# istellartech/GELATO

Measured on AMD Instinct MI355X. Metric: residual+Jacobian evals/sec (and ms/eval), 6-phase x 64-node LGR mesh, higher is better.
Workload: dtype f64

## Files before the change

gelato_amd/csrc/gel_eval_kernel.h:

```cpp
#pragma once

namespace gel {

enum ParkSlot { PK_Q0 = 0, PK_Q1, PK_Q2, PK_Q3, PK_V0, PK_V1, PK_V2, PK_DJJ, PK_LV0, PK_LV1, PK_LV2,
                PK_FP0, PK_FP1, PK_FP2, PK_FP3, PK_FP4, PK_FP5, PK_FP6, PK_FP7, PK_COUNT };
constexpr int kStageLd = 17;
constexpr int kWaveLds = PK_COUNT * 64;
static_assert(kWaveLds >= 64 * kStageLd, "the MFMA staging tile must fit the wave's park region");
constexpr int kCoopStageOff = PK_LV0 * 64;
static_assert(kWaveLds - kCoopStageOff >= 64 * 11, "the cooperative hand-over area must fit behind the early park slots");
constexpr int kXldsPipeFrom = kLongPhaseFrom;
constexpr int kSlabRowsMax = 68, kPackRows = 36, kParkRes = (PK_LV2 + 1) * 64;
constexpr int kPipeSlabK = 8;
constexpr int wave_lds_doubles(bool jac, bool mfma, bool pack, bool split = false, bool longp = true) {
  return jac ? kWaveLds : (!mfma ? kParkRes : (split ? 64 * kStageLd  : (pack ? kParkRes + 4 * 64  : (longp ? 2 * 4 * kPipeSlabK * 11 + 64 * kPipeSlabK  : kSlabRowsMax * 11))));
}
static_assert(wave_lds_doubles(false, true, false, true) >= kParkRes, "residual-only split form: park over the result tile");
static_assert(wave_lds_doubles(false, true, true) >= 64 * 11 && wave_lds_doubles(false, true, false) >= 64 * 11 && wave_lds_doubles(false, true, false, false, false) >= 64 * 11, "hand-over area");
static_assert(wave_lds_doubles(false, true, true) >= kParkRes && wave_lds_doubles(false, true, false) >= kParkRes && wave_lds_doubles(false, true, false, false, false) >= kParkRes, "residual-only park");

constexpr int kSlotPT = 0, kSlotVM = 3, kSlotVP = 6;

#ifndef GEL_MIN_WAVES_PER_SIMD
#define GEL_MIN_WAVES_PER_SIMD 4
// ... 560 lines not shown
          __builtin_amdgcn_s_barrier();
        }
#undef GEL_PIPE_ROWS
#undef GEL_PIPE_A
#undef GEL_PIPE_WAIT
        lds_double* wg_lds = regions + kHO;
#pragma unroll
        for (int ct = 0; ct < 3; ct++) {
          const int c = 16 * ct + c16;
          const int vb = h7 ? c / 7 : c / 11, col = c - ncv * vb;
          if (c < ncols && (ct < 2 || !h7)) {
#pragma unroll
            for (int i = 0; i < 4; i++) wg_lds[vb * kWL + (16 * wv + kq + 4 * i) * 11 + col] = acc[ct][i];
          }
        }
        __syncthreads();
        if (ghost) return;
        lds_double* row = wave_lds + kHO + lane * 11;
        lm = row[0];
#pragma unroll
        for (int c = 0; c < 3; c++) { lr[c] = row[1 + c]; lv[c] = row[4 + c]; }
#pragma unroll
        for (int c = 0; c < 4; c++) lq[c] = row[7 + c];
      } else if (MFMA && csplit) {
        const int c16 = lane & 15, kq = lane >> 4;
        const double* bp = xm + ph.xa;
        int bs = 1;
        if (c16 >= 1 && c16 < 4) { bp = xr + 3 * ph.xa + (c16 - 1); bs = 3; }
        if (c16 >= 4 && c16 < 7) { bp = xv + 3 * ph.xa + (c16 - 4); bs = 3; }
        if (c16 >= 7) { bp = xq + 4 * ph.xa + ((c16 < 11) ? (c16 - 7) : 0); bs = 4; }
        gel_double4 acc1 = gel_double4{0.0, 0.0, 0.0, 0.0};
        const double* ap1 = P.Dst + (size_t)dsw * 4 + part * 64 + lane;
        const unsigned un = (unsigned)n, ubs = (unsigned)bs;
        if (tail1 && rb) {
          xl[0] = xm[ph.xa + n];
#pragma unroll
          for (int c = 0; c < 3; c++) { xl[1 + c] = xr[3 * (ph.xa + n) + c]; xl[4 + c] = xv[3 * (ph.xa + n) + c]; }
#pragma unroll
          for (int c = 0; c < 4; c++) xl[7 + c] = xq[4 * (ph.xa + n) + c];
        }
        constexpr int kSplitB = SPLITB, kSplitA = 4;
        if (n < kSlabRowsMax) {
          static_assert(!(SPLIT && MFMA && !JAC) || kSlabRowsMax * 11 <= kWL, "the state-row image must fit a wavefront's region");
          lds_double* img = wave_lds + (1 - part) * kWL;
          constexpr int kQRows = kSlabRowsMax / 4, kQ = kQRows * 11;
#pragma unroll
          for (int i = 0; i < (kQ + 63) / 64; i++) {
            const int e = lane + 64 * i;
            const int rl = (e * 373) >> 12, c = e - 11 * rl;
            const int r = kQRows * part + rl;
            if (e < kQ) {
              const int xr_ = ph.xa + min(r, n);
              const int off = (c == 0) ? xr_ : ((c < 4) ? M + 3 * xr_ + (c - 1) : ((c < 7) ? 4 * M + 3 * xr_ + (c - 4) : 7 * M + 4 * xr_ + (c - 7)));
              const double v = xb[off];
              img[r * 11 + c] = (r <= n) ? v : 0.0;
            }
          }
          double a1[kSplitA];
#pragma unroll
          for (int i = 0; i < kSplitA; i++) a1[i] = ap1[min(i, ksteps - 1) * 256];
          __syncthreads();
          const int bo = kq * 11 + ((c16 < 11) ? c16 : 0);
#pragma unroll
          for (int i = 0; i < kSlabRowsMax / 4; i++) {
            if (i < ksteps) {
              acc1 = __builtin_amdgcn_mfma_f64_16x16x4f64(a1[i % kSplitA], img[bo + 44 * i], acc1, 0, 0, 0);
              a1[i % kSplitA] = ap1[min(i + kSplitA, ksteps - 1) * 256];
            }
          }
        } else {
          for (int k0 = 0; k0 < ksteps; k0 += kSplitB) {
            double bl[kSplitB], a1[kSplitA];
#pragma unroll
            for (int i = 0; i < kSplitB; i++) bl[i] = bp[min(4u * (k0 + i) + kq, un) * ubs];
#pragma unroll
            for (int i = 0; i < kSplitA; i++) a1[i] = ap1[min(k0 + i, ksteps - 1) * 256];
#pragma unroll
            for (int i = 0; i < kSplitB; i++) {
              if (k0 + i < ksteps) {
                acc1 = __builtin_amdgcn_mfma_f64_16x16x4f64(a1[i % kSplitA], bl[i], acc1, 0, 0, 0);
                a1[i % kSplitA] = ap1[min(k0 + i + kSplitA, ksteps - 1) * 256];
              }
            }
          }
        }
        lds_double* lead_lds = wave_lds - part * kWL;
#pragma unroll
        for (int i = 0; i < 4; i++) lead_lds[(16 * part + kq + 4 * i) * kStageLd + c16] = acc1[i];
        __syncthreads();
        if (only_dx) return;
        if (rb) {
          lds_double* row = wave_lds + lane * kStageLd;
          lm = row[0];
#pragma unroll
          for (int c = 0; c < 3; c++) { lr[c] = row[1 + c]; lv[c] = row[4 + c]; }
#pragma unroll
          for (int c = 0; c < 4; c++) lq[c] = row[7 + c];
        }
      } else if (MFMA) {
        const int c16 = lane & 15, kq = lane >> 4;
        const double* bp = xm + ph.xa;
        int bs = 1;
        if (c16 >= 1 && c16 < 4) { bp = xr + 3 * ph.xa + (c16 - 1); bs = 3; }
        if (c16 >= 4 && c16 < 7) { bp = xv + 3 * ph.xa + (c16 - 4); bs = 3; }
        if (c16 >= 7) { bp = xq + 4 * ph.xa + ((c16 < 11) ? (c16 - 7) : 0); bs = 4; }
        gel_double4 acc[4];
#pragma unroll
        for (int t = 0; t < 4; t++) acc[t] = gel_double4{0.0, 0.0, 0.0, 0.0};
        const gel_double4* ap = reinterpret_cast<const gel_double4*>(P.Dsw) + (size_t)dsw * 1 + lane;
        const unsigned un = (unsigned)n, ubs = (unsigned)bs;
        if (tail1) {
          xl[0] = xm[ph.xa + n];
#pragma unroll
          for (int c = 0; c < 3; c++) { xl[1 + c] = xr[3 * (ph.xa + n) + c]; xl[4 + c] = xv[3 * (ph.xa + n) + c]; }
#pragma unroll
          for (int c = 0; c < 4; c++) xl[7 + c] = xq[4 * (ph.xa + n) + c];
        }
        constexpr int kSplitB = SPLITB, kSplitA = 2;
        for (int k0 = 0; k0 < ksteps; k0 += kSplitB) {
          double bl[kSplitB];
          gel_double4 a4[kSplitA];
#pragma unroll
          for (int i = 0; i < kSplitB; i++) bl[i] = bp[min(4u * (k0 + i) + kq, un) * ubs];
#pragma unroll
          for (int i = 0; i < kSplitA; i++) a4[i] = ap[min(k0 + i, ksteps - 1) * 64];
#pragma unroll
          for (int i = 0; i < kSplitB; i++) {
            if (k0 + i < ksteps) {
#pragma unroll
              for (int t = 0; t < 4; t++) acc[t] = __builtin_amdgcn_mfma_f64_16x16x4f64(a4[i % kSplitA][t], bl[i], acc[t], 0, 0, 0);
              a4[i % kSplitA] = ap[min(k0 + i + kSplitA, ksteps - 1) * 64];
            }
          }
        }
#pragma unroll
        for (int t = 0; t < 4; t++)
#pragma unroll
          for (int i = 0; i < 4; i++) wave_lds[(16 * t + kq + 4 * i) * kStageLd + c16] = acc[t][i];
        lds_double* row = wave_lds + lane * kStageLd;
        lm = row[0];
#pragma unroll
        for (int c = 0; c < 3; c++) { lr[c] = row[1 + c]; lv[c] = row[4 + c]; }
#pragma unroll
        for (int c = 0; c < 4; c++) lq[c] = row[7 + c];
      } else {
        const double* Dt = P.Dt + ph.doff + j;
        const double* pm = xm + ph.xa;
        const double* pr = xr + 3 * ph.xa;
        const double* pv = xv + 3 * ph.xa;
        const double* pq = xq + 4 * ph.xa;
        for (int i = 0; i <= n; i++) {
          const double d = Dt[(size_t)i * n];
          lm += d * pm[i];
#pragma unroll
          for (int c = 0; c < 3; c++) lr[c] += d * pr[3 * i + c];
#pragma unroll
          for (int c = 0; c < 3; c++) lv[c] += d * pv[3 * i + c];
#pragma unroll
          for (int c = 0; c < 4; c++) lq[c] += d * pq[4 * i + c];
        }
      }
    }
    GEL_TAKE_KNOT_TIMES();
#undef GEL_DX_TAIL_ACC
    if (SPLIT && tail1 && rb) {
      lm = __builtin_fma(dlast, xl[0], lm);
#pragma unroll
      for (int c = 0; c < 3; c++) { lr[c] = __builtin_fma(dlast, xl[1 + c], lr[c]); lv[c] = __builtin_fma(dlast, xl[4 + c], lv[c]); }
#pragma unroll
      for (int c = 0; c < 4; c++) lq[c] = __builtin_fma(dlast, xl[7 + c], lq[c]);
    }
    if (MFMA && !active) return;
    PARK_SET(PK_Q0, q[0]); PARK_SET(PK_Q1, q[1]); PARK_SET(PK_Q2, q[2]); PARK_SET(PK_Q3, q[3]);
    PARK_SET(PK_V0, ve[0]); PARK_SET(PK_V1, ve[1]); PARK_SET(PK_V2, ve[2]);
    if (JAC) PARK_SET(PK_DJJ, djj);
    if (rb) { PARK_SET(PK_LV0, lv[0]); PARK_SET(PK_LV1, lv[1]); PARK_SET(PK_LV2, lv[2]); }
    if (!ref0_done) {
      if (rb && !ph.engine_on) m0 = xm[ph.xa];
      if (rb && ph.hold) {
#pragma unroll
        for (int c = 0; c < 4; c++) q0[c] = xq[4 * ph.xa + c];
      }
    }

    if (JAC && lead) {
      if (coo) {
        const double sc = -(P.kpt * (tf - to));
        double* d_ = P.coo_full + GEL_COO_BASE(CG_PV) + (size_t)3 * j0;
#pragma unroll
        for (int i = 0; i < 3; i++) d_[(cw8 == 512) ? 64 * i + lane : 3 * lane + i] = sc;
      } else if (j == 0) EMIT_AT(packed ? (ph.K - sub_hi) * cw8 : ph.K * n * 8, -(P.kpt * (tf - to)));
      {
        const double pt[3] = {ve[0] * P.kpt, ve[1] * P.kpt, ve[2] * P.kpt};
        EMIT_GROUP(3, kSlotPT, pt, CG_PT, 0, true, true);
      }
    }
    if (!ph.hold && lead) {
      double fq[4];
      quat_rate(q, u0, u1, P.uu, fq);
      if (rb) {
        double cq[4];
#pragma unroll
        for (int c = 0; c < 4; c++) cq[c] = lq[c] - fq[c] * (tf - to) * hT;
        RSTORE_ROWS(wave_lds + kTileOff, 4, rs_q, cq);
      }
      if (JAC && ph.q_fd) {
        double f[4];
#pragma unroll
        for (int k = 0; k < 4; k++) {
          double qp[4];
#pragma unroll
          for (int c = 0; c < 4; c++) qp[c] = (k == c) ? (q[c] + dx) : q[c];
          quat_rate(qp, u0, u1, P.uu, f);
          const int c0 = (k < 2) ? 2 : 0;
          EMIT(ph.s_qq + 2 * k, FDQ(f[c0], fq[c0]));
          EMIT(ph.s_qq + 2 * k + 1, FDQ(f[c0 + 1], fq[c0 + 1]));
        }
#pragma unroll 1
        for (int k = 0; k < 2; k++) {
          quat_rate(q, (k == 0) ? u0 + dx : u0, (k == 1) ? u1 + dx : u1, P.uu, f);
#pragma unroll
          for (int c = 0; c < 4; c++) EMIT(ph.s_qq + 8 + 4 * k + c, FDQ(f[c], fq[c]));
        }
#pragma unroll
        for (int c = 0; c < 4; c++) EMIT(ph.s_qq + 16 + c, fq[c] * hT);
      } else if (JAC) {
        const double hS = (tf - to) * ut / 2.0;
        const double d2r = 0.017453292519943295769;
        EMIT(ph.s_qq + 0, 0.5 * ((u0 * P.uu) * d2r) * hS);
        EMIT(ph.s_qq + 1, 0.5 * ((u1 * P.uu) * d2r) * hS);
        const double kq = 0.5 * (P.uu * d2r) * hS;
        if (coo) {
          const double C0 = kq * q[0], C1 = kq * q[1], C2 = kq * q[2], C3 = kq * q[3];
          const double u0v[4] = {C2, C3, -C0, -C1}, u1v[4] = {C3, -C2, C1, -C0};
          EMIT_GROUP(4, 0, u0v, CG_QU, 0, false, true);
          EMIT_GROUP(4, 0, u1v, CG_QU, 1, false, true);
        } else {
          EMIT(ph.s_qq + 2, -(kq * q[0]));
          EMIT(ph.s_qq + 3, kq * q[1]);
          EMIT(ph.s_qq + 4, kq * q[2]);
          EMIT(ph.s_qq + 5, kq * q[3]);
        }
        {
          const double qt[4] = {fq[0] * hT, fq[1] * hT, fq[2] * hT, fq[3] * hT};
          EMIT_GROUP(4, ph.s_qq + 6, qt, CG_QT, 0, true, true);
        }
      }
    }
    if (rb) {
      double cm;
      if (ph.engine_on) {
        const double rh = ph.mf_um * (tf - to) * ut / 2.0;
        cm = lm - rh;
      } else {
        cm = me - m0;
      }
      RSTORE(rs_m + gn, cm);
      GEL_CHK(cm);
      {
        double cp[3];
        const double kpos = P.kpt * (tf - to);
#pragma unroll
        for (int c = 0; c < 3; c++) cp[c] = lr[c] - ve[c] * kpos;
        RSTORE_ROWS(wave_lds + kTileOff, 3, rs_p, cp);
      }
      if (ph.hold) {
        double cq[4];
#pragma unroll
        for (int c = 0; c < 4; c++) cq[c] = q[c] - q0[c];
        RSTORE_ROWS(wave_lds + kTileOff, 4, rs_q, cq);
      }
    }
  }
  asm volatile("" ::: "memory");

  double fc[3];
  {
    const double tn = tau * (tf - to) / 2 + (tf + to) / 2;
    const double inv_m = frcp(me * P.um);

#define GEL_QUAT_CLOSED(Tval)                                                                                          \
  do {                                                                                                                 \
    const double kq_ = ((Tval) * inv_m) * (inv_uv * fds);                                                              \
    const double q_[4] = {PARK_GET(PK_Q0), PARK_GET(PK_Q1), PARK_GET(PK_Q2), PARK_GET(PK_Q3)};                         \
    _Pragma("unroll") for (int k = 0; k < 4; k++) {                                                                    \
      const double dl_ = (q_[k] + dx) - q_[k];                                                                         \
      const double a_ = (k < 2) ? -(dl_ * kq_) : dl_ * kq_;    \
      const double b_ = -2.0 * (dl_ * kq_);                                                                            \
      const double vq_[3] = {(2.0 * q_[k] + dl_) * a_,                                                                 \
                             q_[3 - k] * b_,                                    \
                             ((k & 1) ? q_[k ^ 2] : -q_[k ^ 2]) * b_};        \
      EMIT_GROUP(3, ph.s_vq + 3 * k, vq_, CG_VQ, k, false, true);                                                      \
    }                                                                                                                  \
  } while (0)
#define GEL_MASS_CLOSED(tm_)                                                                                           \
  do {                                                                                                                 \
          \
    const double e_ = (fresh_product(me + dx, P.um) - fresh_product(me, P.um)) * inv_m;                                \
    const double k_ = (e_ * (1.0 - e_ * (1.0 - e_))) * (inv_uv * fds);                                                 \
    const double vm_[3] = {(tm_)[0] * k_, (tm_)[1] * k_, (tm_)[2] * k_};                                               \
    EMIT_GROUP(3, kSlotVM, vm_, CG_VM, 0, false, true);                                                                \
  } while (0)
    if (ph.air) {
      EarthHalf eh{1.0, 0.0};
      bool have_eh = false;
#define GEL_NEED_EARTH_ANGLE(wn_, we_)                                                                                 \
  do {                                                                                                                 \
    if (!have_eh && __builtin_amdgcn_ballot_w64(!((wn_) == 0.0 && (we_) == 0.0)) != 0) {                                \
      int jl_ = jc;                                                                                                    \
      if (AERO) asm volatile("" : "+v"(jl_));    \
      const double tau_ = P.tau[ph.toff + jl_];                                                                        \
      const EarthAngle e_ = earth_angle(tau_ * (tf - to) / 2 + (tf + to) / 2);                                         \
      eh.ch = e_.ch; eh.sh = e_.sh; have_eh = true;                                                                    \
    }                                                                                                                  \
  } while (0)
      PosCentreTail pt;
      double cen_rho = 0.0, cen_P = 0.0, cen_inv_a = 0.0;
      double dir2 = 0.0;
      EarthHalf aeh{1.0, 0.0};
      bool have_aeh = false;
#ifndef GEL_AEH
#define GEL_AEH aeh
#endif
#ifndef GEL_X_NOPOS
#define GEL_X_NOPOS 0
#endif
#ifndef GEL_X_NOQUAT
#define GEL_X_NOQUAT 0
#endif
#ifndef GEL_X_NOVEL
#define GEL_X_NOVEL 0
#endif
      const bool aero_on = AERO && akinds != 0;
      const bool a_need_alpha = AERO && (akinds & 5) != 0;
#define GEL_AERO_NEED_EA(wn_, we_)                                                                                     \
  do {                                                                                                                 \
    if (!have_aeh && __builtin_amdgcn_ballot_w64(!((wn_) == 0.0 && (we_) == 0.0)) != 0) {                               \
      int jl_ = jc;                                                                                                    \
      asm volatile("" : "+v"(jl_));    \
      const double tau_ = P.tau[ph.toff + jl_];                                                                        \
      const EarthAngle e_ = earth_angle((tau_ * (tf - to) / 2 + (tf + to) / 2) * P.ut);                                \
      aeh.ch = e_.ch; aeh.sh = e_.sh; have_aeh = true;                                                                 \
    }                                                                                                                  \
  } while (0)
#define GEL_AERO_FETCH()                                                                                               \
  const int ab_[3] = {load_const(&aph->base[0]), load_const(&aph->base[1]), load_const(&aph->base[2])};                \
  const double ax_[3] = {load_const(&aph->ilx[0]), load_const(&aph->ilx[1]), load_const(&aph->ilx[2])};                \
  const int n8_ = 8 * n, j08_ = 8 * j0
#define GEL_AERO_ENTRY(blk, col, a_, nv2_, d_, ind_, rho_, okl_, a_cc, a_ac, a_qc, a_isc, a_ok)                         \
  do {                                                                                                                 \
    double t_ = 0.0, dq_ = 0.0, qp_ = 0.0;                                                                             \
    const double ac_ = a_ac;                                                                                           \
    {                                                                                                                  \
      const double qc_ = a_qc;                                                                                         \
      qp_ = 0.5 * (rho_) * (nv2_);                                                                                     \
      dq_ = qp_ - qc_;                                                                                                 \
      if (a_need_alpha) {                                                                                              \
        const double cp_ = aero_cos(a_, nv2_, d_, ind_);                                                               \
        const bool okd_ = aero_dalpha(cp_, nv2_, a_cc, a_isc, a_ok, t_);                                               \
        if (__builtin_amdgcn_ballot_w64(!okd_) != 0) {                                                                 \
          const double t2_ = aero_acos(cp_, nv2_) - ac_;                                                               \
          t_ = okd_ ? t_ : t2_;                                                                                        \
        }                                                                                                              \
      }                                                                                                                \
    }                                                                                                                  \
    _Pragma("unroll") for (int kind = 0; kind < 3; kind++) {                                                           \
      if ((blk) == 2 && kind == 1) continue;                             \
      const double df_ = (kind == 0) ? t_ : ((kind == 1) ? dq_ : qp_ * t_ + dq_ * ac_);                                \
      const double gv = -(df_ * ax_[kind]);                                                                            \
      if (okl_) AEMIT(ab_[kind] + (((blk) == 0 ? 1 : ((blk) == 1 ? 4 : 7)) + (col)) * n8_ + j08_, gv);                 \
    }                                                                                                                  \
  } while (0)
#if GEL_CA_CACHE
      Bracket ca_br = no_bracket();
#define GEL_CA_BRACKET (JAC ? &ca_br : (Bracket*)nullptr)
#else
#define GEL_CA_BRACKET nullptr
#endif
      struct ParkSink { lds_double* park; GEL_DEV void put(int i, double v) const { if (!(AERO && (i == PCS_P || i == PCS_IH))) park[(PK_FP0 + i) * 64] = v; } };
      constexpr int PK_ACC = PK_FP0 + PCS_P, PK_AAC = PK_FP0 + PCS_IH, PK_AQC = PK_LV2;
      static_assert(PCS_COUNT == 8 && PK_FP7 == PK_FP0 + 7, "PosCentre's early members fill FP0-7");
      {
        PosPart pp;
        double v[3], w[3], F[3], dir[3];
        const double r[3] = {fresh_product(re[0], P.up), fresh_product(re[1], P.up), fresh_product(re[2], P.up)};
        if (JAC) pp = pos_part<true, ParkSink>(r, tb, P.barC20, nullptr, ParkSink{park}, &pt);
        else pp = pos_part(r, tb, P.barC20);
        if (__builtin_amdgcn_ballot_w64(!(pp.wn == 0.0 && pp.we == 0.0)) != 0) {
          const EarthAngle e0 = earth_angle(tn);
          eh.ch = e0.ch; eh.sh = e0.sh; have_eh = true;
          if (aero_on) PARK_SET(PK_ACC, tn);
        }
        const EarthAngle ea = full_angle(eh);
        wind_eci_or_calm(r, ea, pp.shp, pp.chp, pp.inv_p, pp.wn, pp.we, w);
#pragma unroll
        for (int c = 0; c < 3; c++) v[c] = PARK_GET(PK_V0 + c) * P.uv;
        aero_force(r, v, pp.rho, pp.inv_a, ea, w, ph.area, tb, F, GEL_CA_BRACKET);
#define GEL_T (ph.thrust - ph.nozzle * pp.P)
#define GEL_TDC(name) const double name[3] = {GEL_T * dir[0], GEL_T * dir[1], GEL_T * dir[2]}
        {
          const double q[4] = {PARK_GET(PK_Q0), PARK_GET(PK_Q1), PARK_GET(PK_Q2), PARK_GET(PK_Q3)};
          thrust_dir(q, dir);
        }
        double tm[3];
        {
          GEL_TDC(Tdc);
          accel_parts(Tdc, F, inv_m, pp.g, inv_uv, tm, fc);
        }
        if (rb) {
#ifndef GEL_RES_XPOSE_VEL_AIR
#define GEL_RES_XPOSE_VEL_AIR 1
#endif
          if (!JAC || GEL_RES_XPOSE_VEL_AIR) {
            double cv[3];
#pragma unroll
            for (int c = 0; c < 3; c++) cv[c] = PARK_GET(PK_LV0 + c) - fc[c] * (tf - to) * hT;
            RSTORE_ROWS(wave_lds + PK_LV0 * 64, 3, rs_v, cv);
          } else {
#pragma unroll
            for (int c = 0; c < 3; c++) {
              const double cv = PARK_GET(PK_LV0 + c) - fc[c] * (tf - to) * hT;
              RSTORE(rs_v + 3 * gn + c, cv);
              GEL_CHK(cv);
            }
          }
        }
        if (JAC) {
          asm volatile("" ::: "memory");
          PARK_SET(PK_LV0, pp.shp); PARK_SET(PK_LV1, pp.chp);
          if (!AERO) PARK_SET(PK_LV2, pp.inv_p);
        }
        if (JAC && lead && !P.fd_recompute) GEL_MASS_CLOSED(tm);
        if (JAC && ph.air_fd && (SPLIT && P.split_vel ? !lead : lead)) {
          double f[3];
          {
            const double djj = PARK_GET(PK_DJJ);
#pragma unroll
            for (int k = 0; k < 3; k++) {
              if (SPLIT && P.split_vel && k != part - 1) continue;
              double vp[3], Fp[3];
#pragma unroll
              for (int c = 0; c < 3; c++) vp[c] = ((k == c) ? (PARK_GET(PK_V0 + c) + dx) : PARK_GET(PK_V0 + c)) * P.uv;
              const double r[3] = {fresh_product(re[0], P.up), fresh_product(re[1], P.up), fresh_product(re[2], P.up)};
              aero_force(r, vp, pp.rho, pp.inv_a, ea, w, ph.area, tb, Fp, GEL_CA_BRACKET);
              GEL_TDC(Tdc);
              accel(Tdc, Fp, inv_m, pp.g, inv_uv, f);
#pragma unroll
              for (int c = 0; c < 3; c++) EMIT(ph.s_vv + 3 * k + c, ((c == k) ? djj : 0.0) + FDQ(f[c], fc[c]));
            }
          }
        }
        if (JAC && lead) {
          double f[3];
          if (!P.fd_recompute) {
            GEL_QUAT_CLOSED(GEL_T);
          } else if (P.fd_recompute) {
            const double q[4] = {PARK_GET(PK_Q0), PARK_GET(PK_Q1), PARK_GET(PK_Q2), PARK_GET(PK_Q3)};
#pragma unroll 1
            for (int k = 0; k < 4; k++) {
              double qp[4];
#pragma unroll
              for (int c = 0; c < 4; c++) qp[c] = (k == c) ? (q[c] + dx) : q[c];
              double dp[3];
              thrust_dir(qp, dp);
              const double Td[3] = {GEL_T * dp[0], GEL_T * dp[1], GEL_T * dp[2]};
              accel(Td, F, inv_m, pp.g, inv_uv, f);
#pragma unroll
              for (int c = 0; c < 3; c++) EMIT(ph.s_vq + 3 * k + c, FDQ(f[c], fc[c]));
            }
            GEL_TDC(Tdc);
            accel(Tdc, F, frcp((me + dx) * P.um), pp.g, inv_uv, f);
#pragma unroll
            for (int c = 0; c < 3; c++) EMIT(kSlotVM + c, FDQ(f[c], fc[c]));
          }
          if (!ph.t_fd) {
            const double vt[3] = {fc[0] * hT, fc[1] * hT, fc[2] * hT};
            EMIT_GROUP(3, ph.s_vt, vt, CG_VT, 0, true, true);
          }
        }
        if (aero_on) {
          asm volatile("" ::: "memory");
          const double ra[3] = {fresh_product(re[0], P.up), fresh_product(re[1], P.up), fresh_product(re[2], P.up)};
          double va[3], wa[3], a0[3];
#pragma unroll
          for (int c = 0; c < 3; c++) va[c] = PARK_GET(PK_V0 + c) * P.uv;
          if (have_eh) {
            const EarthAngle e1 = earth_angle(PARK_GET(PK_ACC) * P.ut);
            aeh.ch = e1.ch; aeh.sh = e1.sh; have_aeh = true;
          }
          if (have_aeh) {
            PosCentre pcx;
            double wn_, we_, p_, ip_, ih_;
            pos_centre_tail(pt, pp.rho, pp.P, tb, pcx, wn_, we_);
            geodetic_p_ih(ra[0], ra[1], ra[2], p_, ip_, ih_);
            wind_eci(ra, full_angle(GEL_AEH), PARK_GET(PK_LV0), PARK_GET(PK_LV1), ip_, wn_, we_, wa);
          } else {
            wa[0] = 0.0; wa[1] = 0.0; wa[2] = 0.0;
          }
          const double nv2 = aero_vair2(ra, va, wa, a0);
          const double ind = frsqrt(fmax(dir[0] * dir[0] + dir[1] * dir[1] + dir[2] * dir[2], 1.0e-300));
          const double cc = a_need_alpha ? aero_cos(a0, nv2, dir, ind) : 0.0;
          const double alpha_c = a_need_alpha ? aero_acos(cc, nv2) : 0.0;
          const double qdyn_c = 0.5 * pp.rho * nv2;
          double sc, isc;
          fsqrt_rsqrt(fmax((1.0 - cc) * (1.0 + cc), 1.0e-300), sc, isc);
          const bool centre_ok = (cc <= 1.0) && (nv2 >= 1.0e-12) && (sc > 1.0e-6);
          GEL_AERO_FETCH();
          const double ail_[3] = {load_const(&aph->il[0]), load_const(&aph->il[1]), load_const(&aph->il[2])};
#pragma unroll
          for (int kind = 0; kind < 3; kind++) {
            const double il = ail_[kind];
            const double cv = 1.0 - ((kind == 0) ? alpha_c : (kind == 1) ? qdyn_c : qdyn_c * alpha_c) * il;
            AEMIT(ab_[kind] + j08_, cv);
            GEL_CHK(cv);
          }
          if (a_need_alpha && !GEL_X_NOQUAT) {
            const double q[4] = {PARK_GET(PK_Q0), PARK_GET(PK_Q1), PARK_GET(PK_Q2), PARK_GET(PK_Q3)};
#pragma unroll
            for (int c = 0; c < 4; c++) {
              double qp[4], dp[3];
#pragma unroll
              for (int d = 0; d < 4; d++) qp[d] = (d == c) ? q[d] + dx : q[d];
              thrust_dir(qp, dp);
              const double indp = frsqrt(fmax(dp[0] * dp[0] + dp[1] * dp[1] + dp[2] * dp[2], 1.0e-300));
              GEL_AERO_ENTRY(2, c, a0, nv2, dp, indp, pp.rho, true, cc, alpha_c, qdyn_c, isc, centre_ok);
              __builtin_amdgcn_sched_barrier(0);
            }
          }
#pragma unroll
          for (int c = 0; c < (GEL_X_NOVEL ? 0 : 3); c++) {
            double vp[3], a[3];
#pragma unroll
            for (int d = 0; d < 3; d++) vp[d] = ((d == c) ? PARK_GET(PK_V0 + d) + dx : PARK_GET(PK_V0 + d)) * P.uv;
            const double nv2p = aero_vair2(ra, vp, wa, a);
            GEL_AERO_ENTRY(1, c, a, nv2p, dir, ind, pp.rho, true, cc, alpha_c, qdyn_c, isc, centre_ok);
            __builtin_amdgcn_sched_barrier(0);
          }
          PARK_SET(PK_ACC, cc); PARK_SET(PK_AAC, centre_ok ? alpha_c : -alpha_c); PARK_SET(PK_AQC, qdyn_c);
        }
        if (JAC) {
          asm volatile("" ::: "memory");
          PARK_SET(PK_Q0, fc[0]); PARK_SET(PK_Q1, fc[1]); PARK_SET(PK_Q2, fc[2]); PARK_SET(PK_Q3, dir[0]); PARK_SET(PK_DJJ, dir[1]);
          dir2 = dir[2];
          cen_rho = pp.rho; cen_P = pp.P; cen_inv_a = pp.inv_a;
        }
#undef GEL_TDC
#undef GEL_T
      }
      if (JAC && (!SPLIT || part)) {
        const int k0 = SPLIT ? part - 1 : 0, k1 = SPLIT ? part : 3;
#define GEL_POS_SWEEP_F(rp, pq, f_)                                                                           \
  do {                                                                                                        \
    double wq_[3], Fp_[3];                                                                                    \
    GEL_NEED_EARTH_ANGLE((pq).wn, (pq).we);                                                                   \
    const EarthAngle ea = full_angle(eh);                                                                     \
    wind_eci_or_calm(rp, ea, (pq).shp, (pq).chp, (pq).inv_p, (pq).wn, (pq).we, wq_);                          \
    const double vq_[3] = {PARK_GET(PK_V0) * P.uv, PARK_GET(PK_V1) * P.uv, PARK_GET(PK_V2) * P.uv};           \
    aero_force(rp, vq_, (pq).rho, (pq).inv_a, ea, wq_, ph.area, tb, Fp_, GEL_CA_BRACKET);                     \
    const double Tp_ = ph.thrust - ph.nozzle * (pq).P;                                                        \
    const double Td_[3] = {Tp_ * PARK_GET(PK_Q3), Tp_ * PARK_GET(PK_DJJ), Tp_ * dir2};                        \
    accel(Td_, Fp_, inv_m, (pq).g, inv_uv, f_);                                                               \
  } while (0)
#define GEL_POS_SWEEP_EMIT(kk, f_, okl_)                                                                      \
  do {                                                                                                        \
    const double vp_[3] = {FDQ((f_)[0], PARK_GET(PK_Q0)), FDQ((f_)[1], PARK_GET(PK_Q1)), FDQ((f_)[2], PARK_GET(PK_Q2))}; \
    EMIT_GROUP(3, kSlotVP + 3 * (kk), vp_, CG_VP, kk, false, okl_);                                           \
  } while (0)
#define GEL_AERO_POS(kk, rp, pq, okl_)                                                                        \
  do {                                                                                                        \
    double wq_[3], a_[3];                                                                                     \
    GEL_AERO_NEED_EA((pq).wn, (pq).we);                                                                       \
    wind_eci_or_calm(rp, full_angle(GEL_AEH), (pq).shp, (pq).chp, (pq).inv_p, (pq).wn, (pq).we, wq_);             \
    const double vq_[3] = {PARK_GET(PK_V0) * P.uv, PARK_GET(PK_V1) * P.uv, PARK_GET(PK_V2) * P.uv};           \
    const double nv2_ = aero_vair2(rp, vq_, wq_, a_);                                                         \
    const double dd_[3] = {PARK_GET(PK_Q3), PARK_GET(PK_DJJ), dir2};                                          \
    const double ind_ = frsqrt(fmax(dd_[0] * dd_[0] + dd_[1] * dd_[1] + dd_[2] * dd_[2], 1.0e-300));          \
    const double cc_ = PARK_GET(PK_ACC);                                                                      \
    double sc_, isc_;                                                                                         \
    fsqrt_rsqrt(fmax((1.0 - cc_) * (1.0 + cc_), 1.0e-300), sc_, isc_);                                        \
    const double acs_ = PARK_GET(PK_AAC);    \
    GEL_AERO_FETCH();                                                                                         \
    GEL_AERO_ENTRY(0, kk, a_, nv2_, dd_, ind_, (pq).rho, okl_, cc_, fabs(acs_), PARK_GET(PK_AQC), isc_, !__builtin_signbit(acs_)); \
  } while (0)
#define GEL_LOAD_POS_CENTRE(pc, pcv)                                                                                   \
  PosCentre pc;                                                                                                        \
  pc.ihy = PARK_GET(PK_FP0 + PCS_IHY);                                                                                 \
  pc.sl = PARK_GET(PK_FP0 + PCS_SL); pc.cl = PARK_GET(PK_FP0 + PCS_CL); pc.icl = PARK_GET(PK_FP0 + PCS_ICL);           \
  pc.N = PARK_GET(PK_FP0 + PCS_N); pc.G = PARK_GET(PK_FP0 + PCS_G);                                                    \
  PosPart pcv;                                                                                                         \
  pcv.rho = cen_rho; pcv.P = cen_P; pcv.inv_a = cen_inv_a;                                                             \
  pcv.shp = PARK_GET(PK_LV0); pcv.chp = PARK_GET(PK_LV1);                                                              \
  if (AERO) {                                                                                                          \
    geodetic_p_ih(fresh_product(re[0], P.up), fresh_product(re[1], P.up), fresh_product(re[2], P.up), pc.p, pcv.inv_p, pc.ih); \
  } else {                                                                                                             \
    pc.p = PARK_GET(PK_FP0 + PCS_P); pc.ih = PARK_GET(PK_FP0 + PCS_IH); pcv.inv_p = PARK_GET(PK_LV2);                  \
  }                                                                                                                    \
  pos_centre_tail(pt, cen_rho, cen_P, tb, pc, pcv.wn, pcv.we)
        unsigned todo = 0;
        unsigned long long coo_okm = 0;
        if (P.fd_recompute) {
          todo = ((1u << k1) - 1u) & ~((1u << k0) - 1u);
        } else {
#pragma unroll
          for (int k = k0; k < k1; k++) {
            asm volatile("" ::: "memory");
            GEL_LOAD_POS_CENTRE(pc, pcv);
            const double r[3] = {fresh_product(re[0], P.up), fresh_product(re[1], P.up), fresh_product(re[2], P.up)};
            double rp[3];
#pragma unroll
            for (int c = 0; c < 3; c++) rp[c] = (k == c) ? (re[c] + dx) * P.up : r[c];
            const double dlt = (k == 0) ? rp[0] - r[0] : ((k == 1) ? rp[1] - r[1] : rp[2] - r[2]);
            PosPart pq;
            const bool ok = pos_delta(r, k, dlt, pcv, pc, tb, pq);
            if (coo) coo_okm = __builtin_amdgcn_ballot_w64(ok);
            if (__builtin_amdgcn_ballot_w64(!ok) != 0) {
              todo |= 1u << k;
              if (__builtin_amdgcn_ballot_w64(ok) == 0) continue;
            }
            gravity_eci(rp, P.barC20, pq.g);
            double f[3];
            GEL_POS_SWEEP_F(rp, pq, f);
            GEL_POS_SWEEP_EMIT(k, f, ok);
            if (aero_on && !GEL_X_NOPOS) GEL_AERO_POS(k, rp, pq, ok);
          }
        }
        if (todo) {
#pragma unroll 1
          for (int k = k0; k < k1; k++) {
            if (!((todo >> k) & 1u)) continue;
            asm volatile("" ::: "memory");
            double rp[3];
#pragma unroll
            for (int c = 0; c < 3; c++) rp[c] = fresh_product((k == c) ? re[c] + dx : re[c], P.up);
            bool ok = false;
            if (!P.fd_recompute && coo) {
              ok = ((coo_okm >> lane) & 1ull) != 0;
            } else if (!P.fd_recompute) {
              GEL_LOAD_POS_CENTRE(pc, pcv);
              const double r[3] = {fresh_product(re[0], P.up), fresh_product(re[1], P.up), fresh_product(re[2], P.up)};
              const double dlt = (k == 0) ? rp[0] - r[0] : ((k == 1) ? rp[1] - r[1] : rp[2] - r[2]);
              PosPart pd;
              ok = pos_delta(r, k, dlt, pcv, pc, tb, pd);
            }
            asm volatile("" ::: "memory");
            PosPart pq = pos_part(rp, tb, P.barC20);
            double f[3];
            GEL_POS_SWEEP_F(rp, pq, f);
            GEL_POS_SWEEP_EMIT(k, f, !ok);
            if (aero_on && !GEL_X_NOPOS) GEL_AERO_POS(k, rp, pq, !ok);
          }
        }
#undef GEL_AERO_POS
#undef GEL_LOAD_POS_CENTRE
#undef GEL_NEED_EARTH_ANGLE
#undef GEL_AERO_NEED_EA
#undef GEL_AERO_ENTRY
#undef GEL_AERO_FETCH
#undef GEL_POS_SWEEP_F
#undef GEL_POS_SWEEP_EMIT
      }
      if (JAC && lead && ph.t_fd) {
        asm volatile("" ::: "memory");
        const double fcc[3] = {PARK_GET(PK_Q0), PARK_GET(PK_Q1), PARK_GET(PK_Q2)};
        int jl2 = jc;
        if (AERO) asm volatile("" : "+v"(jl2));
        const double tau2 = P.tau[ph.toff + jl2];
        {
          const double r[3] = {fresh_product(re[0], P.up), fresh_product(re[1], P.up), fresh_product(re[2], P.up)};
          const PosPart p2 = pos_part(r, tb, P.barC20);
          const double T2 = ph.thrust - ph.nozzle * p2.P;
          PARK_SET(PK_FP0, p2.shp); PARK_SET(PK_FP1, p2.chp); PARK_SET(PK_FP2, p2.inv_p); PARK_SET(PK_FP3, p2.wn); PARK_SET(PK_FP4, p2.we);
          PARK_SET(PK_FP5, p2.rho); PARK_SET(PK_FP6, p2.inv_a);
          PARK_SET(PK_LV0, p2.g[0]); PARK_SET(PK_LV1, p2.g[1]); PARK_SET(PK_LV2, p2.g[2]);
          PARK_SET(PK_Q0, T2 * PARK_GET(PK_Q3)); PARK_SET(PK_Q1, T2 * PARK_GET(PK_DJJ)); PARK_SET(PK_Q2, T2 * dir2);
        }
#pragma unroll 1
        for (int k = 0; k < 2; k++) {
          asm volatile("" ::: "memory");
          const double to_p = (k == 0) ? to + dx : to;
          const double tf_p = (k == 1) ? tf + dx : tf;
          const double tnp = tau2 * (tf_p - to_p) / 2 + (tf_p + to_p) / 2;
          const EarthAngle eq = earth_angle(tnp);
          double wq[3], Fp[3], f[3];
          const double rq[3] = {re[0] * P.up, re[1] * P.up, re[2] * P.up};
          wind_eci_or_calm(rq, eq, PARK_GET(PK_FP0), PARK_GET(PK_FP1), PARK_GET(PK_FP2), PARK_GET(PK_FP3), PARK_GET(PK_FP4), wq);
          const double vq[3] = {PARK_GET(PK_V0) * P.uv, PARK_GET(PK_V1) * P.uv, PARK_GET(PK_V2) * P.uv};
          aero_force(rq, vq, PARK_GET(PK_FP5), PARK_GET(PK_FP6), eq, wq, ph.area, tb, Fp, GEL_CA_BRACKET);
          const double Tq[3] = {PARK_GET(PK_Q0), PARK_GET(PK_Q1), PARK_GET(PK_Q2)};
          const double gq[3] = {PARK_GET(PK_LV0), PARK_GET(PK_LV1), PARK_GET(PK_LV2)};
          accel(Tq, Fp, inv_m, gq, inv_uv, f);
#pragma unroll
          for (int c = 0; c < 3; c++)
            EMIT(ph.s_vt + 3 * k + c, (fcc[c] * (tf - to) - f[c] * (tf_p - to_p)) * fdt);
        }
      }
    } else {
      const double T = ph.thrust;
      double dir[3];
      {
        const double q[4] = {PARK_GET(PK_Q0), PARK_GET(PK_Q1), PARK_GET(PK_Q2), PARK_GET(PK_Q3)};
        thrust_dir(q, dir);
      }
      const double Td[3] = {T * dir[0], T * dir[1], T * dir[2]};
      double gc[3];
      {
        const double r[3] = {re[0] * P.up, re[1] * P.up, re[2] * P.up};
        gravity_eci(r, P.barC20, gc);
      }
      double tm[3];
#pragma unroll
      for (int c = 0; c < 3; c++) { tm[c] = Td[c] * inv_m; fc[c] = (tm[c] + gc[c]) * inv_uv; }
      if (rb) {
        double cv[3];
#pragma unroll
        for (int c = 0; c < 3; c++) cv[c] = PARK_GET(PK_LV0 + c) - fc[c] * (tf - to) * hT;
        RSTORE_ROWS(wave_lds + PK_LV0 * 64, 3, rs_v, cv);
      }
      if (JAC) {
        double f[3];
        if (!P.fd_recompute) {
          GEL_MASS_CLOSED(tm);
        } else {
          accel_noair(Td, frcp((me + dx) * P.um), gc, inv_uv, f);
#pragma unroll
          for (int c = 0; c < 3; c++) EMIT(kSlotVM + c, FDQ(f[c], fc[c]));
        }
#pragma unroll
        for (int k = 0; k < 3; k++) {
          double r[3], gp[3];
#pragma unroll
          for (int c = 0; c < 3; c++) r[c] = ((k == c) ? (re[c] + dx) : re[c]) * P.up;
          gravity_eci(r, P.barC20, gp);
          accel_noair(Td, inv_m, gp, inv_uv, f);
          const double vp[3] = {FDQ(f[0], fc[0]), FDQ(f[1], fc[1]), FDQ(f[2], fc[2])};
          EMIT_GROUP(3, kSlotVP + 3 * k, vp, CG_VP, k, false, true);
        }
        if (!P.fd_recompute) {
          GEL_QUAT_CLOSED(T);
        } else {
          const double q[4] = {PARK_GET(PK_Q0), PARK_GET(PK_Q1), PARK_GET(PK_Q2), PARK_GET(PK_Q3)};
#pragma unroll 1
          for (int k = 0; k < 4; k++) {
            double qp[4];
#pragma unroll
            for (int c = 0; c < 4; c++) qp[c] = (k == c) ? (q[c] + dx) : q[c];
            double dp[3];
            thrust_dir(qp, dp);
            const double Tp[3] = {T * dp[0], T * dp[1], T * dp[2]};
            accel_noair(Tp, inv_m, gc, inv_uv, f);
#pragma unroll
            for (int c = 0; c < 3; c++) EMIT(ph.s_vq + 3 * k + c, FDQ(f[c], fc[c]));
          }
        }
        {
          const double vt[3] = {fc[0] * hT, fc[1] * hT, fc[2] * hT};
          EMIT_GROUP(3, ph.s_vt, vt, CG_VT, 0, true, true);
        }
      }
    }
  }
#undef EMIT_GROUP
#undef GEL_COO_EMIT
#undef GEL_COO_BASE
#undef EMIT
#undef GEL_CA_BRACKET
#undef GEL_QUAT_CLOSED
#undef GEL_MASS_CLOSED
#undef AEMIT
#undef EMIT_AT
#undef RSTORE
#undef RSTORE_ROWS
#undef RSTORE_LINE
#undef xpose
#undef FDQ
#undef GEL_CHK
#undef GEL_UNI
#undef GEL_TAKE_KNOT_TIMES
#undef PARK_GET
#undef PARK_SET
  if (bad) *(volatile int32_t*)P.flag = 1;
}

__device__ __forceinline__ void signal_done(const ProblemDev& P) {
  if (!P.done_flag) return;
  __threadfence_system();
  __syncthreads();
  if (threadIdx.x == 0) {
    const int old = __hip_atomic_fetch_add(P.done_ctr, 1, __ATOMIC_ACQ_REL, __HIP_MEMORY_SCOPE_AGENT);
    if (old == P.done_total - 1) {
      __hip_atomic_store(P.done_ctr, 0, __ATOMIC_RELAXED, __HIP_MEMORY_SCOPE_AGENT);
      __hip_atomic_store(P.done_flag, P.done_seq, __ATOMIC_RELEASE, __HIP_MEMORY_SCOPE_SYSTEM);
    }
  }
}

template <bool JAC, bool MFMA, bool SPLIT = false, bool PACK = false, bool LONGP = true, bool NTS = true, bool AERO = false>
__global__ __launch_bounds__(kBlock, (!JAC && PACK) ? GEL_MIN_WAVES_PER_SIMD_RES : ((JAC && PACK) ? GEL_MIN_WAVES_PER_SIMD_PACKJAC : GEL_MIN_WAVES_PER_SIMD)) void eval_kernel(ProblemDev P, int B, const double* __restrict__ x,
                                                      double* __restrict__ res, double* __restrict__ jvar) {
  eval_body<JAC, MFMA, SPLIT, PACK, 9, LONGP, NTS, AERO>(P, B, x, res, jvar, blockIdx.x);
  if constexpr (SPLIT) signal_done(P);
}

}
```

gelato_amd/csrc/gel_kernels.hip:

```cpp
#include <hip/hip_runtime.h>

#include "gel_tables.h"

#include "gel_eval_kernel.h"
namespace gel {

constexpr int kExpandGroup = 8;
__global__ __launch_bounds__(kBlock) void expand_kernel(long long nnz, long long V, int B, const double* __restrict__ cval,
                                                        const int32_t* __restrict__ src,
                                                        const double* __restrict__ jvar, double* __restrict__ full) {
  const int b0 = blockIdx.y * kExpandGroup;
  const int nb = min(kExpandGroup, B - b0);
  const bool even = (nnz & 1) == 0;
  for (long long i = 2 * ((long long)blockIdx.x * kBlock + threadIdx.x); i < nnz; i += 2LL * gridDim.x * kBlock) {
    const bool two = i + 1 < nnz;
    const int s0 = src[i], s1 = two ? src[i + 1] : -1;
    const double c0 = (s0 == -1) ? cval[i] : 0.0, c1 = (two && s1 == -1) ? cval[i + 1] : 0.0;
    const int g0 = (s0 >= 0) ? s0 : -2 - s0, g1 = (s1 >= 0) ? s1 : -2 - s1;
    for (int g = 0; g < nb; g++) {
      const double* jv = jvar + (size_t)(b0 + g) * V;
      double* out = full + (size_t)(b0 + g) * nnz + i;
      const double v0 = (s0 == -1) ? c0 : ((s0 >= 0) ? jv[g0] : -jv[g0]);
      const double v1 = (s1 == -1) ? c1 : ((s1 >= 0) ? jv[g1] : -jv[g1]);
      if (two && (even || ((b0 + g) & 1) == 0)) {
        typedef double gel_d2 __attribute__((ext_vector_type(2)));
        __builtin_nontemporal_store(gel_d2{v0, v1}, reinterpret_cast<gel_d2*>(out));
      } else {
        __builtin_nontemporal_store(v0, out);
        if (two) __builtin_nontemporal_store(v1, out + 1);
      }
    }
  }
}

__global__ __launch_bounds__(kBlock) void update_full_kernel(long long nnz, long long V, int nvar, int B, const int32_t* __restrict__ vdst,
                                                             const int32_t* __restrict__ vsrc, const double* __restrict__ jvar,
                                                             double* __restrict__ full) {
  const int i = blockIdx.x * kBlock + threadIdx.x;
  if (i >= nvar) return;
  const int d = vdst[i], s = vsrc[i];
  const int g = (s >= 0) ? s : -2 - s;
  for (int b = blockIdx.y; b < B; b += gridDim.y) {
    const double v = jvar[(size_t)b * V + g];
    full[(size_t)b * nnz + d] = (s >= 0) ? v : -v;
  }
}
__global__ __launch_bounds__(kBlock) void update_lines_kernel(long long nnz, long long V, int nlines, int B, const int32_t* __restrict__ vline,
                                                              const int32_t* __restrict__ src, const double* __restrict__ cval,
                                                              const double* __restrict__ jvar, double* __restrict__ full) {
  const int t = blockIdx.x * kBlock + threadIdx.x;
  if (t >= 8 * nlines) return;
  const long long i = 8LL * vline[t >> 3] + (t & 7);
  const int s = src[i];
  const double c = (s == -1) ? cval[i] : 0.0;
  const int g = (s >= 0) ? s : -2 - s;
  for (int b = blockIdx.y; b < B; b += gridDim.y) {
    double v = c;
    if (s != -1) { const double w = jvar[(size_t)b * V + g]; v = (s >= 0) ? w : -w; }
    __builtin_nontemporal_store(v, full + (size_t)b * nnz + i);
  }
}
__global__ __launch_bounds__(kBlock) void fill_full_kernel(long long nnz, int B, const double* __restrict__ cval, double* __restrict__ full) {
  for (long long i = (long long)blockIdx.x * kBlock + threadIdx.x; i < nnz; i += (long long)gridDim.x * kBlock) {
    const double c = cval[i];
    for (int b = blockIdx.y; b < B; b += gridDim.y) __builtin_nontemporal_store(c, full + (size_t)b * nnz + i);
  }
}

__global__ void perturb_local_kernel(int nloc, double dx, const double* __restrict__ x, const int32_t* __restrict__ colmap,
                                     double* __restrict__ Xp) {
  const long long t = (long long)blockIdx.x * blockDim.x + threadIdx.x;
  if (t >= (long long)(nloc + 1) * nloc) return;
  const int row = (int)(t / nloc), col = (int)(t - (long long)row * nloc);
  double v = x[colmap[col]];
  if (row == col + 1) v += dx;
  Xp[t] = v;
}

__global__ void quotient_local_kernel(int nloc, int nres, int roff, int nrows, double dx, const double* __restrict__ res,
                                      double* __restrict__ J, long long ldJ, int row0, const int32_t* __restrict__ colmap) {
  __shared__ double tile[32][33];
  const int c0 = blockIdx.x * 32, r0 = blockIdx.y * 32;
  for (int k = threadIdx.y; k < 32; k += blockDim.y) {
    const int c = c0 + k, r = r0 + threadIdx.x;
    if (c < nloc && r < nrows) tile[k][threadIdx.x] = res[(size_t)(c + 1) * nres + roff + r];
  }
  __syncthreads();
  for (int k = threadIdx.y; k < 32; k += blockDim.y) {
    const int r = r0 + k, c = c0 + threadIdx.x;
    if (c < nloc && r < nrows) J[(size_t)(row0 + r) * ldJ + (colmap ? colmap[c] : c)] = (tile[threadIdx.x][k] - res[roff + r]) / dx;
  }
}

struct RhsArgs {
  int n, Kw, Kc;
  const double *mass_e, *pos_e, *vel_e, *quat, *t, *tables;
  double thrust, area, nozzle, um, up, uv, barC20;
  double* out;
};

__global__ void rhs_vel_air_kernel(RhsArgs A) {
  extern __shared__ double lds[];
  ProblemDev P{};
  P.Kw = A.Kw; P.Kc = A.Kc; P.tables = A.tables;
  const Tables tb = stage_tables(P, lds);
  const int i = blockIdx.x * blockDim.x + threadIdx.x;
  if (i >= A.n) return;
  const double m = A.mass_e[i] * A.um;
  const double r[3] = {A.pos_e[3 * i] * A.up, A.pos_e[3 * i + 1] * A.up, A.pos_e[3 * i + 2] * A.up};
  const double v[3] = {A.vel_e[3 * i] * A.uv, A.vel_e[3 * i + 1] * A.uv, A.vel_e[3 * i + 2] * A.uv};
  const double q[4] = {A.quat[4 * i], A.quat[4 * i + 1], A.quat[4 * i + 2], A.quat[4 * i + 3]};
  const PosPart pp = pos_part(r, tb, A.barC20);
  const EarthAngle ea = earth_angle(A.t[i]);
  double w[3], F[3], dir[3], f[3];
  wind_eci(r, ea, pp.shp, pp.chp, pp.inv_p, pp.wn, pp.we, w);
  aero_force(r, v, pp.rho, pp.inv_a, ea, w, A.area, tb, F);
  thrust_dir(q, dir);
  const double T = A.thrust - A.nozzle * pp.P;
  const double Td[3] = {T * dir[0], T * dir[1], T * dir[2]};
  accel(Td, F, 1.0 / m, pp.g, 1.0 / A.uv, f);
  for (int c = 0; c < 3; c++) A.out[3 * i + c] = f[c];
}

__global__ void rhs_vel_noair_kernel(RhsArgs A) {
  const int i = blockIdx.x * blockDim.x + threadIdx.x;
  if (i >= A.n) return;
  const double m = A.mass_e[i] * A.um;
  const double r[3] = {A.pos_e[3 * i] * A.up, A.pos_e[3 * i + 1] * A.up, A.pos_e[3 * i + 2] * A.up};
  const double q[4] = {A.quat[4 * i], A.quat[4 * i + 1], A.quat[4 * i + 2], A.quat[4 * i + 3]};
  double dir[3], g[3], f[3];
  thrust_dir(q, dir);
  gravity_eci(r, A.barC20, g);
  const double Td[3] = {A.thrust * dir[0], A.thrust * dir[1], A.thrust * dir[2]};
  accel_noair(Td, 1.0 / m, g, 1.0 / A.uv, f);
  for (int c = 0; c < 3; c++) A.out[3 * i + c] = f[c];
}

__global__ void rhs_quat_kernel(int n, const double* quat, const double* u_e, double unit_u, double* out) {
  const int i = blockIdx.x * blockDim.x + threadIdx.x;
  if (i >= n) return;
  const double q[4] = {quat[4 * i], quat[4 * i + 1], quat[4 * i + 2], quat[4 * i + 3]};
  double dq[4];
  quat_rate(q, u_e[2 * i], u_e[2 * i + 1], unit_u, dq);
  for (int c = 0; c < 4; c++) out[4 * i + c] = dq[c];
}

__global__ void point_kernel(int kind, int n, const double* in, const double* aux, int aux_rows, double* out) {
  extern __shared__ double lds[];
  const int naux = (kind == 5 || kind == 10) ? 3 * aux_rows + 2 * (aux_rows - 1)
                   : (kind == 6 || kind == 9) ? 2 * aux_rows + (aux_rows - 1) : (kind == 0 ? kAtmDoubles : 0);
  for (int i = threadIdx.x; i < naux; i += blockDim.x) lds[i] = aux[i];
  __syncthreads();
  const int i = blockIdx.x * blockDim.x + threadIdx.x;
  if (i >= n) return;
  switch (kind) {
    case 0: {
      const double h = geopotential_altitude(in[i]);
      const Air a = atmosphere(h, lds);
      out[5 * i] = h; out[5 * i + 1] = a.T; out[5 * i + 2] = a.P; out[5 * i + 3] = a.rho; out[5 * i + 4] = a.a;
    } break;
    case 1: {
      double lat, sl, cl, p, ip;
      geodetic_lat_p(in[3 * i], in[3 * i + 1], in[3 * i + 2], lat, p, ip);
      geodetic_sincos_p(in[3 * i], in[3 * i + 1], in[3 * i + 2], sl, cl, p, ip);
      const double lon = atan2(in[3 * i + 1], in[3 * i]);
      out[3 * i] = lat * 180.0 / kPi; out[3 * i + 1] = lon * 180.0 / kPi;
      out[3 * i + 2] = geodetic_alt_from(p, sl, cl);
    } break;
    case 2: {
      const double r[3] = {in[3 * i], in[3 * i + 1], in[3 * i + 2]};
      double g[3];
      gravity_eci(r, aux[0], g);
      out[3 * i] = g[0]; out[3 * i + 1] = g[1]; out[3 * i + 2] = g[2];
    } break;
    case 3: {
      const double* a = in + 6 * i;
      const double r[3] = {a[0], a[1], a[2]};
      double sl, cl, p, ip, w[3];
      geodetic_sincos_p(r[0], r[1], r[2], sl, cl, p, ip);
      const EarthAngle ea = earth_angle(a[3]);
      double chp, irt;
      fsqrt_rsqrt(0.5 * (1.0 + cl), chp, irt);
      wind_eci(r, ea, (0.5 * sl) * irt, chp, ip, a[4], a[5], w);
      out[3 * i] = w[0]; out[3 * i + 1] = w[1]; out[3 * i + 2] = w[2];
    } break;
    case 4: {
      const double* a = in + 7 * i;
      double s, c;
      sincos(kOmega * a[6], &s, &c);
      const double d0 = a[0] - (0.0 * a[5] - kOmega * a[4]);
      const double d1 = a[1] - (kOmega * a[3] - 0.0 * a[5]);
      const double d2 = a[2] - (0.0 * a[4] - 0.0 * a[3]);
      out[3 * i] = d0 * c + d1 * s; out[3 * i + 1] = -d0 * s + d1 * c; out[3 * i + 2] = d2;
    } break;
    case 5: {
      double wn, we;
      wind_ned2(in[i], lds, lds + 3 * aux_rows, aux_rows, wn, we);
      out[3 * i] = wn; out[3 * i + 1] = we; out[3 * i + 2] = 0.0;
    } break;
    case 6: out[i] = interp_tab(in[i], lds, lds + 2 * aux_rows, aux_rows, 2, 1); break;
    case 7: {
      const double a = in[2 * i], b = in[2 * i + 1];
      out[4 * i] = fsqrt(a); out[4 * i + 1] = sqrt(a); out[4 * i + 2] = fdiv(a, b); out[4 * i + 3] = a / b;
    } break;
    case 8: {
      double s1, c1, s2, c2;
      fsincos(in[2 * i], &s1, &c1);
      sincos(in[2 * i], &s2, &c2);
      out[6 * i] = s1; out[6 * i + 1] = c1; out[6 * i + 2] = s2; out[6 * i + 3] = c2;
      out[6 * i + 4] = flog_ratio(in[2 * i + 1]); out[6 * i + 5] = log(in[2 * i + 1]);
    } break;
    case 9: {
      Bracket br = no_bracket();
      for (int k = 0; k < 8; k++) out[8 * i + k] = interp_tab_cached(in[8 * i + k], lds, lds + 2 * aux_rows, aux_rows, 2, 1, br);
    } break;
    case 10: {
      Bracket2 br = no_bracket2();
      for (int k = 0; k < 8; k++) {
        double wn, we;
        wind_ned2_cached(in[8 * i + k], lds, lds + 3 * aux_rows, aux_rows, wn, we, br);
        out[16 * i + 2 * k] = wn; out[16 * i + 2 * k + 1] = we;
      }
    } break;
    case 11: {
      double o[4];
      quatmult(in + 8 * i, in + 8 * i + 4, o);
      for (int c = 0; c < 4; c++) out[4 * i + c] = o[c];
    } break;
    case 12: {
      double o[3];
      quatrot(in + 7 * i, in + 7 * i + 4, o);
      for (int c = 0; c < 3; c++) out[3 * i + c] = o[c];
    } break;
    case 13: {
      const double* q = in + 4 * i;
      out[7 * i] = q[0]; out[7 * i + 1] = -q[1]; out[7 * i + 2] = -q[2]; out[7 * i + 3] = -q[3];
      double d[3];
      thrust_dir(q, d);
      for (int c = 0; c < 3; c++) out[7 * i + 4 + c] = d[c];
    } break;
    case 14: out[2 * i] = fexp(in[i]); out[2 * i + 1] = exp(in[i]); break;
    default: break;
  }
}

struct AeroPos {
  double rho;
  double wn, we;
  double shp, chp, inv_p;
};

GEL_DEV AeroPos aero_pos_part(const double r[3], const Tables& tb) {
  AeroPos o;
  double lat, p, sl, cl;
  geodetic_lat_p(r[0], r[1], r[2], lat, p, o.inv_p);
  fsincos(lat, &sl, &cl);
  const double h = geopotential_altitude(geodetic_alt_from(p, sl, cl));
  wind_ned2(h, tb.wind, tb.winds, tb.Kw, o.wn, o.we);
  double irt;
  fsqrt_rsqrt(0.5 * (1.0 + cl), o.chp, irt);
  o.shp = (0.5 * sl) * irt;
  o.rho = atmosphere(h, tb.atm).rho;
  return o;
}

GEL_DEV double aero_vair(const double r[3], const double v[3], const EarthAngle& ea, const double w[3], double a[3]) {
  const double d0 = v[0] + kOmega * r[1], d1 = v[1] - kOmega * r[0];
  const double e0 = d0 * ea.c + d1 * ea.s, e1 = -d0 * ea.s + d1 * ea.c;
  a[0] = (e0 * ea.c - e1 * ea.s) - w[0]; a[1] = (e0 * ea.s + e1 * ea.c) - w[1]; a[2] = v[2] - w[2];
  return sqrt(a[0] * a[0] + a[1] * a[1] + a[2] * a[2]);
}

GEL_DEV double aero_alpha(const double a[3], double nv, const double q[4]) {
  double dir[3];
  thrust_dir(q, dir);
  const double nd = sqrt(dir[0] * dir[0] + dir[1] * dir[1] + dir[2] * dir[2]);
  const double c_alpha = (a[0] / nv) * (dir[0] / nd) + (a[1] / nv) * (dir[1] / nd) + (a[2] / nv) * (dir[2] / nd);
  return (c_alpha > 1.0) ? 0.0 : ((nv < 1e-6) ? 0.0 : acos(c_alpha));
}

struct AeroOut {
  double* con[3];
  double* jac[3];
  int32_t nrows[3];
  int64_t ld;
  int32_t sm;
};

#ifndef GEL_AERO_UNROLL
#define GEL_AERO_UNROLL 1
#endif
constexpr int kAeroWaves = 4;
enum { AP_ILIM = 0, AP_AC = 3, AP_QC, AP_CC, AP_IS, AP_IND, AP_W = 8, AP_A0 = 11, AP_DIR = 14, AP_RHO = 17, AP_NV2 = 18, AP_INTS = 19,
       kAeroParkSlots = 25 };
typedef __attribute__((address_space(3))) int lds_int;
typedef __attribute__((address_space(3))) double lds_f64;
template <bool ROLES, bool WIDE = false, bool SM = false>
__device__ __forceinline__ void aero_body(const ProblemDev P, int nnodes, const AeroNodeDev* __restrict__ nodes, int tiles, int B,
                                          const double* __restrict__ x, const AeroOut O, const unsigned vblk) {
  extern __shared__ double lds[];
  const Tables tb = stage_tables(P, lds);
  const int lane = (int)(threadIdx.x & 63);
  const int sw = ROLES ? (int)(threadIdx.x >> 6) : -1;
  const long long wid = ROLES ? (long long)vblk : (long long)vblk * kAeroWaves + __builtin_amdgcn_readfirstlane((int)(threadIdx.x >> 6));
  const bool flat = !ROLES && !WIDE && tiles == 0;
  int b, ni_raw;
  bool live;
  if (WIDE) {
    const long long total = (long long)B * nnodes, f = wid * 64 + lane;
    if (wid * 64 >= total) return;
    live = f < total;
    const long long fc = live ? f : total - 1;
    b = (int)(fc / nnodes);
    ni_raw = live ? (int)(fc - (long long)b * nnodes) : nnodes;
  } else if (flat) {
    const long long total = (long long)B * nnodes, f0 = wid * 64;
    if (f0 >= total) return;
    const int b0 = (int)(f0 / nnodes), r0 = (int)(f0 - (long long)b0 * nnodes);
    const bool wrap = r0 + lane >= nnodes;
    live = f0 + lane < total;
    b = live ? (wrap ? b0 + 1 : b0) : b0;
    ni_raw = live ? (wrap ? r0 + lane - nnodes : r0 + lane) : nnodes;
  } else {
    if (wid >= (long long)B * tiles) return;
    b = (int)(wid / tiles);
    ni_raw = (int)(wid - (long long)b * tiles) * 64 + lane;
    live = ni_raw < nnodes;
  }
  const int ni = live ? ni_raw : nnodes - 1;
  const AeroNodeDev Nd = nodes[ni];
  const PhaseDev& ph = P.phases[Nd.phase];
  const double* xb = x + (size_t)b * P.nvars;
  const int M = P.M, N = P.N, xi = ph.xa + Nd.k;
  const double dx = P.dx;
  double re[3];
#pragma unroll
  for (int c = 0; c < 3; c++) re[c] = xb[M + 3 * xi + c];
  const bool want_jac = O.jac[0] || O.jac[1] || O.jac[2];
  const bool need_alpha = __builtin_amdgcn_ballot_w64(live && ((O.con[0] && Nd.row[0] >= 0) || (O.con[2] && Nd.row[2] >= 0))) != 0;
  lds_f64* park = (lds_f64*)lds + ((table_doubles(P.Kw, P.Kc) + 1) & ~1) + (size_t)(threadIdx.x >> 6) * (kAeroParkSlots * 64) + lane;
  lds_int* ipark = (lds_int*)(park - lane + AP_INTS * 64) + lane;
#define AP_AIDX(kind, w) ((kind) == 0 ? ((w) == 3 ? 3 : ((w) == 4 ? 4 : 5)) : ((kind) == 1 ? ((w) == 3 ? 6 : 7) : ((w) == 3 ? 8 : ((w) == 4 ? 9 : 10))))
#define AP_GET(i) (park[(i) * 64])
#define AP_SET(i, v) (park[(i) * 64] = (v))
  PosCentre pc;
  PosPart pp;
  EarthAngle ea{1.0, 0.0, 1.0, 0.0};
  bool have_ea = false;
#define GEL_AERO_NEED_EA(wn_, we_)                                                                                     \
  do {                                                                                                                 \
    if (!have_ea && __builtin_amdgcn_ballot_w64(!((wn_) == 0.0 && (we_) == 0.0)) != 0) {                                \
      const int kn_ = nodes[ni].k, phn_ = nodes[ni].phase;                                                             \
      const double to_ = xb[11 * M + 2 * N + phn_], tf_ = xb[11 * M + 2 * N + phn_ + 1];                               \
      const double tau_ = (kn_ == 0) ? 0.0 : P.tau[P.phases[phn_].toff + kn_ - 1];                                     \
         \
      ea = earth_angle(((kn_ == 0) ? to_ : (tau_ * (tf_ - to_) / 2 + (tf_ + to_) / 2)) * P.ut);                         \
      have_ea = true;                                                                                                  \
    }                                                                                                                  \
  } while (0)
  double chk = 0.0;
  {
    double r[3], v[3], q[4], w[3], a0[3], dir[3];
#pragma unroll
    for (int c = 0; c < 3; c++) { r[c] = re[c] * P.up; v[c] = xb[4 * M + 3 * xi + c] * P.uv; }
#pragma unroll
    for (int c = 0; c < 4; c++) q[c] = xb[7 * M + 4 * xi + c];
    PosCentreTail pt;
    pp = pos_part<true, PosCentreSink, false>(r, tb, 0.0, nullptr, PosCentreSink{&pc}, &pt);
    pos_centre_tail(pt, pp.rho, pp.P, tb, pc, pp.wn, pp.we);
    GEL_AERO_NEED_EA(pp.wn, pp.we);
    wind_eci_or_calm(r, ea, pp.shp, pp.chp, pp.inv_p, pp.wn, pp.we, w);
    const double nv2 = aero_vair2(r, v, w, a0);
    thrust_dir(q, dir);
    const double ind = frsqrt(fmax(dir[0] * dir[0] + dir[1] * dir[1] + dir[2] * dir[2], 1.0e-300));
    const double cc = need_alpha ? aero_cos(a0, nv2, dir, ind) : 0.0;
    const double alpha_c = need_alpha ? aero_acos(cc, nv2) : 0.0;
    const double qdyn_c = 0.5 * pp.rho * nv2;
    double sc, isc;
    fsqrt_rsqrt(fmax((1.0 - cc) * (1.0 + cc), 1.0e-300), sc, isc);
    const bool centre_ok = (cc <= 1.0) && (nv2 >= 1.0e-12) && (sc > 1.0e-6);
#pragma unroll
    for (int kind = 0; kind < 3; kind++) {
      const double il = frcp(Nd.limit[kind]);
      AP_SET(AP_ILIM + kind, il * P.inv_dx);
      const int row = Nd.row[kind];
      {
        const bool has = live && O.jac[kind] && row >= 0;
        const unsigned vb = flat ? (unsigned)b * (unsigned)(O.ld ? (int)O.ld * 8 : O.nrows[kind] * (8 + ((kind == 1) ? 0 : 4)) * 8) : 0u;
        ipark[kind * 64] = 8 * Nd.nk[kind];
        ipark[AP_AIDX(kind, 3) * 64] = has ? (int)(vb + 8u * (unsigned)((SM ? 1 : 3) * Nd.row0[kind] + Nd.ko)) : -1;
        ipark[AP_AIDX(kind, 2) * 64] = has ? (int)(vb + 8u * (unsigned)((SM ? 1 : 2) * Nd.row0[kind] + Nd.ko)) : -1;
        if (kind != 1) ipark[AP_AIDX(kind, 4) * 64] = has ? (int)(vb + 8u * (unsigned)((SM ? 1 : 4) * Nd.row0[kind] + Nd.ko)) : -1;
      }
      if (!live || row < 0 || !O.con[kind] || (ROLES && sw != 0)) continue;
      const double cv = 1.0 - ((kind == 0) ? alpha_c : (kind == 1) ? qdyn_c : qdyn_c * alpha_c) * il;
      if (ROLES) __builtin_nontemporal_store(cv, O.con[kind] + (size_t)b * O.nrows[kind] + row);
      else if (WIDE) O.con[kind][(size_t)b * O.ld + row] = cv;
      else O.con[kind][(size_t)b * (O.ld ? (size_t)O.ld : (size_t)O.nrows[kind]) + row] = cv;
      chk += cv;
    }
    ipark[11 * 64] = centre_ok ? 1 : 0;
    AP_SET(AP_AC, alpha_c); AP_SET(AP_QC, qdyn_c); AP_SET(AP_CC, cc); AP_SET(AP_IS, isc); AP_SET(AP_IND, ind);
#pragma unroll
    for (int c = 0; c < 3; c++) { AP_SET(AP_W + c, w[c]); AP_SET(AP_A0 + c, a0[c]); AP_SET(AP_DIR + c, dir[c]); }
    AP_SET(AP_RHO, pp.rho); AP_SET(AP_NV2, nv2);
  }
#define GEL_AERO_EMIT(boff, width, col, a, nv2, d, ind, rho, skip_q, zero, skip_lane)                                      \
  do {                                                                                                            \
    double t_ = 0.0, dq_ = 0.0, qp_ = 0.0;                                                                        \
    const double ac_ = AP_GET(AP_AC);                                                                             \
    if (!(zero)) {                                                                                                \
      const double qc_ = AP_GET(AP_QC);                                                                           \
      qp_ = 0.5 * (rho) * (nv2);                                                                                  \
      dq_ = qp_ - qc_;                                                                                            \
      if (need_alpha) {                                                                                           \
        const double cp_ = aero_cos(a, nv2, d, ind);                                                              \
        const bool okd_ = aero_dalpha(cp_, nv2, AP_GET(AP_CC), AP_GET(AP_IS), ipark[11 * 64] != 0, t_);           \
        if (__builtin_amdgcn_ballot_w64(!okd_) != 0) {                                                            \
          const double t2_ = aero_acos(cp_, nv2) - ac_;                                                           \
          t_ = okd_ ? t_ : t2_;                                                                                   \
        }                                                                                                         \
      }                                                                                                           \
    }                                                                                                             \
    _Pragma("unroll") for (int kind = 0; kind < 3; kind++) {                                                      \
      if ((skip_q) && kind == 1) continue;                         \
      const int a8_ = ipark[AP_AIDX(kind, width) * 64];                                                           \
      if (a8_ == -1 || (skip_lane)) continue;                                                                     \
      if (SM && (zero)) continue;                           \
      const int nq = (kind == 1) ? 0 : 4;                                                                         \
      const int bo = ((boff) < 0) ? (6 + nq) : (boff);                                                            \
      const double df_ = (kind == 0) ? t_ : ((kind == 1) ? dq_ : qp_ * t_ + dq_ * ac_);                           \
      const double gv = (zero) ? 0.0 : -(df_ * AP_GET(AP_ILIM + kind));                                           \
      gel_au2 gd_;                                                                                                \
      __builtin_memcpy(&gd_, &gv, 8);                                                                             \
      if (WIDE) O.jac[kind][(size_t)b * O.ld + (size_t)bo * O.nrows[kind] + ((a8_ + (col) * ipark[kind * 64]) >> 3)] = gv;                     \
      else if (SM) __builtin_amdgcn_raw_buffer_store_b64(gd_, jrs[kind], a8_ + ((((boff) < 0) ? 11 : ((boff) == 0 ? 1 : ((boff) == 3 ? 4 : 7))) + (col)) * ipark[kind * 64], 0, 0); \
      else __builtin_amdgcn_raw_buffer_store_b64(gd_, jrs[kind], ((col) == 0) ? a8_ : a8_ + (col) * ipark[kind * 64], 8 * bo * O.nrows[kind], ROLES ? 2 : 0);  \
      chk += gv;                                                                                                  \
    }                                                                                                             \
  } while (0)
  typedef unsigned gel_au2 __attribute__((ext_vector_type(2)));
  __amdgpu_buffer_rsrc_t jrs[3];
#pragma unroll
  for (int kind = 0; kind < 3; kind++)
    jrs[kind] = __builtin_amdgcn_make_buffer_rsrc((O.jac[kind] && !WIDE) ? (void*)(O.jac[kind] + (flat ? (size_t)0 : (size_t)__builtin_amdgcn_readfirstlane(b) * (O.ld ? (size_t)O.ld : (size_t)O.nrows[kind] * (8 + ((kind == 1) ? 0 : 4))))) : (void*)nullptr,
                                                  0, -1, 0x00020000);
  if (want_jac) {
#pragma unroll 1
    for (int c = (ROLES && sw != 0) ? 2 : 0; c < 2; c++) {
      if (P.fd_recompute) {
        const int kn = nodes[ni].k, phn = nodes[ni].phase;
        const double to2 = xb[11 * M + 2 * N + phn], tf2 = xb[11 * M + 2 * N + phn + 1];
        const double tau2 = (kn == 0) ? 0.0 : P.tau[P.phases[phn].toff + kn - 1];
        const double to_p = (c == 0) ? to2 + dx : to2, tf_p = (c == 1) ? tf2 + dx : tf2;
        const double tp = ((kn == 0) ? to_p : (tau2 * (tf_p - to_p) / 2 + (tf_p + to_p) / 2)) * P.ut;
        const EarthAngle eq = earth_angle(tp);
        const double r[3] = {fresh_product(re[0], P.up), fresh_product(re[1], P.up), fresh_product(re[2], P.up)};
        const double vq[3] = {xb[4 * M + 3 * xi] * P.uv, xb[4 * M + 3 * xi + 1] * P.uv, xb[4 * M + 3 * xi + 2] * P.uv};
        double wq[3], aq[3];
        wind_eci(r, eq, pp.shp, pp.chp, pp.inv_p, pp.wn, pp.we, wq);
        const double nvq = aero_vair2(r, vq, wq, aq);
        const double dq[3] = {AP_GET(AP_DIR), AP_GET(AP_DIR + 1), AP_GET(AP_DIR + 2)};
        GEL_AERO_EMIT(-1, 2, c, aq, nvq, dq, AP_GET(AP_IND), pp.rho, false, false, false);
      } else {
        const double none[3] = {0.0, 0.0, 0.0};
        GEL_AERO_EMIT(-1, 2, c, none, 0.0, none, 0.0, 0.0, false, true, false);
      }
    }
#define GEL_AERO_POS_TAIL(c, rp, pq, skip_)                                                          \
  do {                                                                                               \
    double wq_[3], a_[3];                                                                            \
    GEL_AERO_NEED_EA((pq).wn, (pq).we);                                                              \
    wind_eci_or_calm(rp, ea, (pq).shp, (pq).chp, (pq).inv_p, (pq).wn, (pq).we, wq_);                 \
    const double vq_[3] = {xb[4 * M + 3 * xi] * P.uv, xb[4 * M + 3 * xi + 1] * P.uv, xb[4 * M + 3 * xi + 2] * P.uv}; \
    const double nv2_ = aero_vair2(rp, vq_, wq_, a_);                                                \
    const double dd_[3] = {AP_GET(AP_DIR), AP_GET(AP_DIR + 1), AP_GET(AP_DIR + 2)};                  \
    GEL_AERO_EMIT(0, 3, c, a_, nv2_, dd_, AP_GET(AP_IND), (pq).rho, false, false, skip_);                  \
  } while (0)
    const unsigned mine = ROLES ? ((sw == 0) ? 0u : (1u << (sw - 1))) : 7u;
    unsigned todo = P.fd_recompute ? mine : 0u;
    unsigned bad = P.fd_recompute ? 7u : 0u;
    if (!P.fd_recompute) {
#if GEL_AERO_UNROLL
#pragma unroll
#else
#pragma unroll 1
#endif
      for (int c = 0; c < 3; c++) {
        if (!((mine >> c) & 1u)) continue;
        asm volatile("" ::: "memory");
        const double r[3] = {fresh_product(re[0], P.up), fresh_product(re[1], P.up), fresh_product(re[2], P.up)};
        double rp[3];
#pragma unroll
        for (int d = 0; d < 3; d++) rp[d] = (d == c) ? (re[d] + dx) * P.up : r[d];
        const double dlt = (c == 0) ? rp[0] - r[0] : ((c == 1) ? rp[1] - r[1] : rp[2] - r[2]);
        PosPart pq;
        const bool okp = pos_delta(r, c, dlt, pp, pc, tb, pq);
        if (__builtin_amdgcn_ballot_w64(!okp) != 0) { todo |= 1u << c; if (!okp) bad |= 1u << c; }
        GEL_AERO_POS_TAIL(c, rp, pq, !okp);
      }
    }
    if (todo) {
      asm volatile("" ::: "memory");
#pragma unroll 1
      for (int c = 0; c < 3; c++) {
        if (!((todo >> c) & 1u)) continue;
        double rp[3];
#pragma unroll
        for (int d = 0; d < 3; d++) rp[d] = ((d == c) ? xb[M + 3 * xi + d] + dx : xb[M + 3 * xi + d]) * P.up;
        const PosPart pf = pos_part<false, NoSink, false>(rp, tb, 0.0);
        GEL_AERO_POS_TAIL(c, rp, pf, !((bad >> c) & 1u));
      }
    }
#undef GEL_AERO_POS_TAIL
    asm volatile("" ::: "memory");
#if GEL_AERO_UNROLL
#pragma unroll
#else
#pragma unroll 1
#endif
    for (int c = (ROLES && sw != 0) ? 3 : 0; c < 3; c++) {
      double vp[3], a[3];
      const double r[3] = {xb[M + 3 * xi] * P.up, xb[M + 3 * xi + 1] * P.up, xb[M + 3 * xi + 2] * P.up};
#pragma unroll
      for (int d = 0; d < 3; d++) vp[d] = ((d == c) ? xb[4 * M + 3 * xi + d] + dx : xb[4 * M + 3 * xi + d]) * P.uv;
      const double wc[3] = {AP_GET(AP_W), AP_GET(AP_W + 1), AP_GET(AP_W + 2)};
      const double dc[3] = {AP_GET(AP_DIR), AP_GET(AP_DIR + 1), AP_GET(AP_DIR + 2)};
      const double nv2 = aero_vair2(r, vp, wc, a);
      GEL_AERO_EMIT(3, 3, c, a, nv2, dc, AP_GET(AP_IND), AP_GET(AP_RHO), false, false, false);
    }
    if (need_alpha && !(ROLES && sw != 0)) {
#if GEL_AERO_UNROLL
#pragma unroll
#else
#pragma unroll 1
#endif
      for (int c = 0; c < 4; c++) {
        double qp[4], dp[3];
#pragma unroll
        for (int d = 0; d < 4; d++) qp[d] = (d == c) ? xb[7 * M + 4 * xi + d] + dx : xb[7 * M + 4 * xi + d];
        thrust_dir(qp, dp);
        const double indp = frsqrt(fmax(dp[0] * dp[0] + dp[1] * dp[1] + dp[2] * dp[2], 1.0e-300));
        const double ac[3] = {AP_GET(AP_A0), AP_GET(AP_A0 + 1), AP_GET(AP_A0 + 2)};
        GEL_AERO_EMIT(6, 4, c, ac, AP_GET(AP_NV2), dp, indp, AP_GET(AP_RHO), true, false, false);
      }
    }
  }
#undef GEL_AERO_EMIT
#undef GEL_AERO_NEED_EA
#undef AP_AIDX
#undef AP_GET
#undef AP_SET
  if (!(fabs(chk) <= 1.79769313486231570815e308)) *(volatile int32_t*)P.flag = 1;
}

#ifndef GEL_AERO_MIN_WAVES
#define GEL_AERO_MIN_WAVES 3
#endif
#ifndef GEL_AERO_XCD_RANGES
#define GEL_AERO_XCD_RANGES 1
#endif
__device__ __forceinline__ unsigned aero_xcd_block(unsigned p, unsigned n) {
  const unsigned n8 = n >> 3;
  return (GEL_AERO_XCD_RANGES && p < 8u * n8) ? (p & 7u) * n8 + (p >> 3) : p;
}
__global__ __launch_bounds__(64 * kAeroWaves, GEL_AERO_MIN_WAVES) void aero_kernel(ProblemDev P, int nnodes, const AeroNodeDev* __restrict__ nodes,
                                                                int tiles, int B, const double* __restrict__ x, AeroOut O) {
  aero_body<false>(P, nnodes, nodes, tiles, B, x, O, aero_xcd_block(blockIdx.x, gridDim.x));
}
__global__ __launch_bounds__(64 * kAeroWaves, GEL_AERO_MIN_WAVES) void aero_sm_kernel(ProblemDev P, int nnodes, const AeroNodeDev* __restrict__ nodes,
                                                                   int tiles, int B, const double* __restrict__ x, AeroOut O) {
  aero_body<false, false, true>(P, nnodes, nodes, tiles, B, x, O, aero_xcd_block(blockIdx.x, gridDim.x));
}
__global__ __launch_bounds__(64 * kAeroWaves, 2) void aero_wide_kernel(ProblemDev P, int nnodes, const AeroNodeDev* __restrict__ nodes,
                                                                int B, const double* __restrict__ x, AeroOut O) {
  aero_body<false, true>(P, nnodes, nodes, 0, B, x, O, blockIdx.x);
}

hipError_t launch_aero_wide(const ProblemDev& P, int nnodes, const AeroNodeDev* nodes, int B, const double* d_x,
                            const AeroLaunchOut& out, long long ld, hipStream_t s) {
  if (B <= 0 || nnodes <= 0) return hipSuccess;
  AeroOut O;
  for (int k = 0; k < 3; k++) { O.con[k] = out.con[k]; O.jac[k] = out.jac[k]; O.nrows[k] = out.nrows[k]; }
  O.ld = ld; O.sm = 0;
  const size_t lds = sizeof(double) * (((staged_table_doubles(P.Kw, P.Kc) + 1) & ~(size_t)1) + (size_t)kAeroWaves * kAeroParkSlots * 64);
  const long long waves = ((long long)B * nnodes + 63) / 64;
  hipLaunchKernelGGL(aero_wide_kernel, dim3((unsigned)((waves + kAeroWaves - 1) / kAeroWaves)), dim3(64 * kAeroWaves), lds, s, P, nnodes, nodes, B, d_x, O);
  return hipGetLastError();
}

AeroForm aero_form(int nnodes, int B, const int32_t* nrows, long long ld) {
  AeroForm f{false, 1, B, 0};
  if (B <= 0 || nnodes <= 0) return f;
  const bool flat_shape = B > 1 && nnodes >= 64 && (nnodes & 63) != 0;
  if (ld > 0 && flat_shape) {
    const long long run = ((1LL << 32) - (1LL << 25)) / (ld * 8);
    if (run >= 1 && run < B) { f.runs = (B + run - 1) / run; f.run_len = run; }
  }
  for (int k = 0; k < 3; k++) f.max_bytes = std::max(f.max_bytes, f.run_len * (ld ? ld : (long long)nrows[k] * (8 + ((k == 1) ? 0 : 4))) * 8);
  f.flat = f.run_len > 1 && nnodes >= 64 && (nnodes & 63) != 0 && f.max_bytes < (1LL << 32) - (1LL << 24);
  return f;
}

hipError_t launch_aero(const ProblemDev& P, int nnodes, const AeroNodeDev* nodes, int B, const double* d_x,
                       const AeroLaunchOut& out, hipStream_t s, long long ld, bool spec_major) {
  if (B <= 0 || nnodes <= 0) return hipSuccess;
  const AeroForm form = aero_form(nnodes, B, out.nrows, ld);
  if (form.runs > 1) {
    for (long long b0 = 0; b0 < B; b0 += form.run_len) {
      AeroLaunchOut o = out;
      for (int k = 0; k < 3; k++) { if (o.con[k]) o.con[k] += b0 * ld; if (o.jac[k]) o.jac[k] += b0 * ld; }
      const hipError_t e = launch_aero(P, nnodes, nodes, (int)std::min<long long>(form.run_len, B - b0), d_x + b0 * P.nvars, o, s, ld, spec_major);
      if (e != hipSuccess) return e;
    }
    return hipSuccess;
  }
  AeroOut O;
  for (int k = 0; k < 3; k++) { O.con[k] = out.con[k]; O.jac[k] = out.jac[k]; O.nrows[k] = out.nrows[k]; }
  O.ld = ld; O.sm = (ld > 0 && spec_major) ? 1 : 0;
  int tiles = (nnodes + 63) / 64;
  const size_t lds = sizeof(double) * (((staged_table_doubles(P.Kw, P.Kc) + 1) & ~(size_t)1) + (size_t)kAeroWaves * kAeroParkSlots * 64);
  long long waves = (long long)B * tiles;
  if (form.flat) {
    waves = ((long long)B * nnodes + 63) / 64;
    tiles = 0;
  }
  const unsigned grid = (unsigned)((waves + kAeroWaves - 1) / kAeroWaves);
  if (O.sm) hipLaunchKernelGGL(aero_sm_kernel, dim3(grid), dim3(64 * kAeroWaves), lds, s, P, nnodes, nodes, tiles, B, d_x, O);
  else hipLaunchKernelGGL(aero_kernel, dim3(grid), dim3(64 * kAeroWaves), lds, s, P, nnodes, nodes, tiles, B, d_x, O);
  return hipGetLastError();
}

GEL_DEV void iip_faa(const double pe[3], const double ve[3], double& lat_deg, double& lon_deg) {
  const double a = 6378137.0, f = 1.0 / 298.257223563, b = a * (1.0 - f), e2 = 2.0 * f - f * f;
  lat_deg = 0.0; lon_deg = 0.0;
  double r_k1 = b;
  const double r0 = sqrt(pe[0] * pe[0] + pe[1] * pe[1] + pe[2] * pe[2]);
  if (r0 < r_k1) return;
  const double vi[3] = {ve[0] - kOmega * pe[1], ve[1] + kOmega * pe[0], ve[2]};
  const double v0 = sqrt(vi[0] * vi[0] + vi[1] * vi[1] + vi[2] * vi[2]);
  const double eps_cos = (r0 * (v0 * v0) / kMu) - 1.0;
  if (eps_cos >= 1.0) return;
  const double a_t = r0 / (1.0 - eps_cos);
  const double eps_sin = (pe[0] * vi[0] + pe[1] * vi[1] + pe[2] * vi[2]) / sqrt(kMu * a_t);
  const double eps2 = eps_cos * eps_cos + eps_sin * eps_sin;
  if (sqrt(eps2) <= 1.0 && a_t * (1.0 - sqrt(eps2)) - a >= 0.0) return;
  double Ek = 0.0, Fk = 0.0, Gk = 0.0, r_k2 = 0.0, r_prev = 0.0, eps_k_sin = 0.0, dcos = 0.0, dsin = 0.0;
  const double root = sqrt((a_t * a_t * a_t) / kMu);
  for (int it = 0; it < 5; it++) {
    const double eps_k_cos = (a_t - r_k1) / a_t;
    if (eps2 - eps_k_cos * eps_k_cos < 0.0) return;
    eps_k_sin = -sqrt(eps2 - eps_k_cos * eps_k_cos);
    dcos = (eps_k_cos * eps_cos + eps_k_sin * eps_sin) / eps2;
    dsin = (eps_k_sin * eps_cos - eps_k_cos * eps_sin) / eps2;
    const double fs = (dcos - eps_cos) / (1.0 - eps_cos);
    const double gs = (dsin + eps_sin - eps_k_sin) * root;
    Ek = fs * pe[0] + gs * vi[0]; Fk = fs * pe[1] + gs * vi[1]; Gk = fs * pe[2] + gs * vi[2];
    const double q = Gk / r_k1;
    r_k2 = a / sqrt((e2 / (1.0 - e2)) * (q * q) + 1.0);
    r_prev = r_k1;
    r_k1 = r_k2;
  }
  if (fabs(r_prev - r_k2) > 1.0) return;
  const double delta = atan2(dsin, dcos);
  const double time_sec = (delta + eps_sin - eps_k_sin) * root;
  const double phi = atan2(tan(asin(Gk / r_k2)), 1.0 - e2);
  const double lam = atan2(Fk, Ek) - kOmega * time_sec;
  lat_deg = phi * 180.0 / kPi;
  lon_deg = lam * 180.0 / kPi;
}

GEL_DEV double distance_vincenty(double lat_o, double lon_o, double lat_t, double lon_t) {
  const double Ra = 6378137.0, f = 1.0 / 298.257223563, Rb = Ra * (1.0 - f);
  const double lat1 = lat_o * kPi / 180.0, lon1 = lon_o * kPi / 180.0, lat2 = lat_t * kPi / 180.0, lon2 = lon_t * kPi / 180.0;
  if (lon2 - lon1 == 0.0) return 0.0;
  const double U1 = atan((1.0 - f) * tan(lat1)), U2 = atan((1.0 - f) * tan(lat2)), dl = lon2 - lon1;
  const double sU1 = sin(U1), cU1 = cos(U1), sU2 = sin(U2), cU2 = cos(U2);
  double lam = dl, sin_sigma = 0.0, cos_sigma = 0.0, sigma = 0.0, cos_alpha = 0.0, cos_2sm = 0.0;
  for (int it = 0; it < 5000; it++) {
    const double sl = sin(lam), cl = cos(lam);
    const double t1 = cU2 * sl, t2 = cU1 * sU2 - sU1 * cU2 * cl;
    sin_sigma = sqrt(t1 * t1 + t2 * t2);
    cos_sigma = sU1 * sU2 + cU1 * cU2 * cl;
    sigma = atan2(sin_sigma, cos_sigma);
    const double sin_alpha = cU1 * cU2 * sl / sin_sigma;
    cos_alpha = sqrt(1.0 - sin_alpha * sin_alpha);
    cos_2sm = cos_sigma - 2.0 * sU1 * sU2 / (cos_alpha * cos_alpha);
    const double coeff = f / 16.0 * (cos_alpha * cos_alpha) * (4.0 + f * (4.0 - 3.0 * (cos_alpha * cos_alpha)));
    const double prev = lam;
    lam = dl + (1.0 - coeff) * f * sin_alpha * (sigma + coeff * sin_sigma * (cos_2sm + coeff * cos_sigma * (-1.0 + 2.0 * cos_2sm)));
    if (fabs(lam - prev) < 1e-12) break;
  }
  const double u2 = (cos_alpha * cos_alpha) * (Ra * Ra - Rb * Rb) / (Rb * Rb);
  const double A = 1.0 + u2 / 16384.0 * (4096.0 + u2 * (-768.0 + u2 * (320.0 - 175.0 * u2)));
  const double Bc = u2 / 1024.0 * (256.0 + u2 * (-128.0 + u2 * (74.0 - 47.0 * u2)));
  const double ds = Bc * sin_sigma * (cos_2sm + 0.25 * Bc * (cos_sigma * (-1.0 + 2.0 * (cos_2sm * cos_2sm)) -
                    (1.0 / 6.0) * Bc * cos_2sm * (-3.0 + 4.0 * (sin_sigma * sin_sigma)) * (-3.0 + 4.0 * (cos_2sm * cos_2sm))));
  return Rb * A * (sigma - ds);
}

GEL_DEV double node_fn(int fn, const double r[3], const double v[3], double t, const double* p) {
  if (fn >= 9) {
    double sn, cs;
    sincos(kOmega * t, &sn, &cs);
    const double pe[3] = {r[0] * cs + r[1] * sn, -r[0] * sn + r[1] * cs, r[2]};
    if (fn <= 11) {
      double lat, lon, alt;
      geodetic_full(pe[0], pe[1], pe[2], lat, lon, alt);
      return (fn == 9) ? lat * (180.0 / kPi) : (fn == 10) ? lon * (180.0 / kPi) : alt;
    }
    if (fn == 15) {
      double lat, lon, alt;
      geodetic_full(pe[0], pe[1], pe[2], lat, lon, alt);
      return distance_vincenty(p[2], p[3], lat * (180.0 / kPi), lon * (180.0 / kPi));
    }
    if (fn <= 13) {
      const double d0 = v[0] + kOmega * r[1], d1 = v[1] - kOmega * r[0];
      const double ve[3] = {d0 * cs + d1 * sn, -d0 * sn + d1 * cs, v[2]};
      double la, lo;
      iip_faa(pe, ve, la, lo);
      return (fn == 12) ? la : lo;
    }
    const double d[3] = {pe[0] - p[2], pe[1] - p[3], pe[2] - p[4]};
    const double dn = sqrt(d[0] * d[0] + d[1] * d[1] + d[2] * d[2]);
    return (d[0] / dn) * p[5] + (d[1] / dn) * p[6] + (d[2] / dn) * p[7];
  }
  const double rn = sqrt(r[0] * r[0] + r[1] * r[1] + r[2] * r[2]);
  const double vn = sqrt(v[0] * v[0] + v[1] * v[1] + v[2] * v[2]);
  if (fn == 0) return 0.5 * vn * vn - kMu / rn;
  if (fn == 7) return rn;
  if (fn == 8) return vn;
  const double c[3] = {r[1] * v[2] - r[2] * v[1], r[2] * v[0] - r[0] * v[2], r[0] * v[1] - r[1] * v[0]};
  const double c2 = c[0] * c[0] + c[1] * c[1] + c[2] * c[2];
  if (fn == 1) return sqrt(c2);
  if (fn == 2) return acos(c[2] / sqrt(c2));
  const double f[3] = {v[1] * c[2] - v[2] * c[1] - kMu * (r[0] / rn), v[2] * c[0] - v[0] * c[2] - kMu * (r[1] / rn),
                       v[0] * c[1] - v[1] * c[0] - kMu * (r[2] / rn)};
  const double e = sqrt(f[0] * f[0] + f[1] * f[1] + f[2] * f[2]) / kMu;
  if (fn == 4) return e;
  const double a = (c2 / kMu) / (1.0 - e * e);
  if (fn == 3) return a;
  return (fn == 5) ? a * (1.0 - e) : a * (1.0 + e);
}

__device__ __forceinline__ void rows_body(const ProblemDev P, int nlin, const LinRowDev* __restrict__ lin, int nfn,
                                          const FnRowDev* __restrict__ fr, int B, int lin_blocks, const double* __restrict__ x,
                                          double* __restrict__ con, double* __restrict__ jfn, const unsigned vblk) {
  const int R = nlin + nfn;
  double chk = 0.0;
  if ((int)vblk < lin_blocks) {
    const long long t = (long long)vblk * blockDim.x + threadIdx.x;
    if (t >= (long long)B * nlin) return;
    const int b = (int)(t / nlin), r = (int)(t - (long long)b * nlin);
    const LinRowDev L = lin[r];
    const double* xb = x + (size_t)b * P.nvars;
    double s = L.coef0 * xb[L.idx0];
    if (L.idx1 >= 0) s += L.coef1 * xb[L.idx1];
    chk = con[(size_t)b * R + r] = s + L.c0;
  } else {
    const long long t = (long long)(vblk - lin_blocks) * blockDim.x + threadIdx.x;
    const long long grp = t >> 3;
    const int sw = (int)(t & 7);
    const bool live = grp < (long long)B * nfn;
    const long long g2 = live ? grp : 0;
    const int b = (int)(g2 / nfn), row = (int)(g2 - (long long)b * nfn);
    const FnRowDev F = fr[row];
    const double* xb = x + (size_t)b * P.nvars;
    double r[3], v[3];
#pragma unroll
    for (int c = 0; c < 3; c++) {
      const double pe = xb[P.M + 3 * F.node + c], ve = xb[4 * P.M + 3 * F.node + c];
      r[c] = ((sw == 1 + c) ? pe + P.dx : pe) * P.up;
      v[c] = ((sw == 4 + c) ? ve + P.dx : ve) * P.uv;
    }
    double tk = 0.0;
    if (F.tcol >= 0) {
      const double te = xb[11 * P.M + 2 * P.N + F.tcol];
      tk = ((sw == 7) ? te + P.dx : te) * P.ut;
    }
    const double f = node_fn(F.fn, r, v, tk, F.p);
    const int vm = F.mode & 3;
    double g = (vm == 0) ? f / F.p[0] - F.p[1] : (f - F.p[1]) / F.p[0];
    if (F.mode & 8) g = -g;
    const int lane0 = (int)(threadIdx.x & 63 & ~7);
    const double gc = __shfl(g, lane0, 64), fc = __shfl(f, lane0, 64);
    if (!live) return;
    if (sw == 0) chk = con[(size_t)b * R + nlin + row] = g;
    else if (jfn) {
      double d;
      if (F.mode & 4) { d = ((f - fc) / P.dx) / F.p[0]; if (F.mode & 8) d = -d; }
      else d = (g - gc) / P.dx;
      chk = jfn[((size_t)b * nfn + row) * 7 + (sw - 1)] = d;
    }
  }
  if (!(fabs(chk) <= 1.79769313486231570815e308)) *(volatile int32_t*)P.flag = 1;
}

__global__ void rows_kernel(ProblemDev P, int nlin, const LinRowDev* __restrict__ lin, int nfn,
                            const FnRowDev* __restrict__ fr, int B, int lin_blocks, const double* __restrict__ x,
                            double* __restrict__ con, double* __restrict__ jfn) {
  rows_body(P, nlin, lin, nfn, fr, B, lin_blocks, x, con, jfn, blockIdx.x);
}

struct CallbackArgs {
  int32_t nb_eval, nb_aero;
  int32_t nnodes, tiles;
  const AeroNodeDev* nodes;
  AeroOut O;
  int32_t nlin, nfn, lin_blocks;
  const LinRowDev* lin;
  const FnRowDev* fr;
  double* con;
  double* jfn;
};
static_assert(64 * kAeroWaves == 256, "callback_kernel's workgroup is the aero workgroup (four roles of one tile)");
template <bool JAC, bool MFMA>
__global__ __launch_bounds__(256) void callback_kernel(ProblemDev P, const double* __restrict__ x, double* __restrict__ res,
                                                       double* __restrict__ jvar, CallbackArgs A) {
  const unsigned b = blockIdx.x;
  if (b < (unsigned)A.nb_eval) eval_body<JAC, MFMA, true, false, 17>(P, 1, x, res, jvar, b);
  else if (b < (unsigned)(A.nb_eval + A.nb_aero)) aero_body<true>(P, A.nnodes, A.nodes, A.tiles, 1, x, A.O, b - (unsigned)A.nb_eval);
  else rows_body(P, A.nlin, A.lin, A.nfn, A.fr, 1, A.lin_blocks, x, A.con, A.jfn, b - (unsigned)(A.nb_eval + A.nb_aero));
  signal_done(P);
}

hipError_t launch_callback(const ProblemDev& P0, bool want_jac, const double* d_x, double* d_res, double* d_jvar,
                           int nnodes, const AeroNodeDev* nodes, const AeroLaunchOut* aero,
                           int nlin, const LinRowDev* lin, int nfn, const FnRowDev* fr, double* d_con, double* d_jfn, hipStream_t s) {
  ProblemDev P = P0;
  P.unit0 = 4 * P0.chunk0;
  P.nunits = 4 * P0.nchunks;
  CallbackArgs A{};
  A.nb_eval = (P.nunits + 3) / 4;
  if (aero && nnodes > 0) {
    for (int k = 0; k < 3; k++) { A.O.con[k] = aero->con[k]; A.O.jac[k] = aero->jac[k]; A.O.nrows[k] = aero->nrows[k]; }
    A.O.ld = 0; A.O.sm = 0;
    A.nnodes = nnodes; A.nodes = nodes; A.tiles = (nnodes + 63) / 64; A.nb_aero = A.tiles;
  }
  int rows_blocks = 0;
  if (d_con && nlin + nfn > 0) {
    A.nlin = nlin; A.nfn = nfn; A.lin = lin; A.fr = fr; A.con = d_con; A.jfn = d_jfn;
    A.lin_blocks = (nlin + 255) / 256;
    rows_blocks = A.lin_blocks + (nfn * 8 + 255) / 256;
  }
  const size_t lds_eval = sizeof(double) * ((size_t)P.park_off + (size_t)wave_lds_doubles(want_jac, P.use_mfma != 0, false, true) * 4);
  const size_t lds_aero = sizeof(double) * (((staged_table_doubles(P.Kw, P.Kc) + 1) & ~(size_t)1) + (size_t)kAeroWaves * kAeroParkSlots * 64);
  const size_t lds = lds_eval > lds_aero ? lds_eval : lds_aero;
  const dim3 grid((unsigned)(A.nb_eval + A.nb_aero + rows_blocks));
  if (P.done_flag) P.done_total = (int32_t)grid.x;
  if (want_jac) {
    if (P.use_mfma) hipLaunchKernelGGL((callback_kernel<true, true>), grid, dim3(256), lds, s, P, d_x, d_res, d_jvar, A);
    else hipLaunchKernelGGL((callback_kernel<true, false>), grid, dim3(256), lds, s, P, d_x, d_res, d_jvar, A);
// ... 327 lines not shown
```

gelato_amd/csrc/gel_kernels_exact.hip:

```cpp
#include <hip/hip_runtime.h>

#include "gel_tables.h"
#include "gel_eval_kernel.h"
#include "gel_exact.h"

namespace gel {

constexpr int kExactBlock = 256;

__global__ __launch_bounds__(kExactBlock) void exact_jac_kernel(ProblemDev P, int B, const double* __restrict__ x,
                                                                double* __restrict__ jvar) {
  extern __shared__ double lds[];
  const Tables tb = stage_tables(P, lds, true);
  const long long t = (long long)blockIdx.x * blockDim.x + threadIdx.x;
  if (t >= (long long)B * P.N) return;
  const int N = P.N, M = P.M;
  const int b = (int)(t / N), g = (int)(t - (long long)b * N);
  const int sec = P.node_phase[g];
  const PhaseDev ph = P.phases[sec];
  const int n = ph.n, j = g - ph.ua;
  const int xj = ph.xa + 1 + j;
  const double* xb = x + (size_t)b * P.nvars;
  const double me = xb[xj];
  const double re[3] = {xb[M + 3 * xj], xb[M + 3 * xj + 1], xb[M + 3 * xj + 2]};
  const double ve[3] = {xb[4 * M + 3 * xj], xb[4 * M + 3 * xj + 1], xb[4 * M + 3 * xj + 2]};
  const double q[4] = {xb[7 * M + 4 * xj], xb[7 * M + 4 * xj + 1], xb[7 * M + 4 * xj + 2], xb[7 * M + 4 * xj + 3]};
  const double u0 = ph.hold ? 0.0 : xb[11 * M + 2 * g], u1 = ph.hold ? 0.0 : xb[11 * M + 2 * g + 1];
  const double to = xb[11 * M + 2 * N + sec], tf = xb[11 * M + 2 * N + sec + 1];
  const double tau = P.tau[ph.toff + j];
  const double djj = P.Dt[ph.doff + (size_t)(j + 1) * n + j];
  const double ut = P.ut, hT = P.hT;
  const double S = (tf - to) * ut / 2.0;
  const double inv_uv = P.inv_uv;

  const int j0 = j & ~63, w = min(64, n - j0);
  double* const out = jvar + (size_t)b * P.V + ph.voff + (size_t)j0 * ph.K + (j - j0);
  bool bad = false;
#define XPUT(slot, val)                                        \
  do {                                                         \
    const double v_ = (val);                                   \
    out[(size_t)(slot) * w] = v_;                              \
    bad = bad || !(fabs(v_) <= 1.79769313486231570815e308);    \
  } while (0)

#pragma unroll
  for (int c = 0; c < 3; c++) XPUT(kSlotPT + c, ve[c] * P.kpt);
  if (j == 0) {
    const double sc = -(P.kpt * (tf - to));
    jvar[(size_t)b * P.V + ph.voff + (size_t)ph.K * n] = sc;
    bad = bad || !(fabs(sc) <= 1.79769313486231570815e308);
  }

  if (!ph.hold) {
    const double hS = (tf - to) * ut / 2.0;
    const double d2r = 0.017453292519943295769;
    XPUT(ph.s_qq + 0, 0.5 * ((u0 * P.uu) * d2r) * hS);
    XPUT(ph.s_qq + 1, 0.5 * ((u1 * P.uu) * d2r) * hS);
    const double kq = 0.5 * (P.uu * d2r) * hS;
    XPUT(ph.s_qq + 2, -(kq * q[0]));
    XPUT(ph.s_qq + 3, kq * q[1]);
    XPUT(ph.s_qq + 4, kq * q[2]);
    XPUT(ph.s_qq + 5, kq * q[3]);
    double fq[4];
    quat_rate(q, u0, u1, P.uu, fq);
#pragma unroll
    for (int c = 0; c < 4; c++) XPUT(ph.s_qq + 6 + c, fq[c] * hT);
  }

  const double tn = tau * (tf - to) / 2 + (tf + to) / 2;
  const double inv_m = frcp(me * P.um);
  const double r[3] = {re[0] * P.up, re[1] * P.up, re[2] * P.up};
  double dir[3];
  thrust_dir(q, dir);
  double T, fc[3], tm[3];
  double dfr[3][3];
  if (ph.air) {
    PosCentre pc;
    PosCentreTail tail;
    const PosPart pp = pos_part<true, PosCentreSink>(r, tb, P.barC20, nullptr, PosCentreSink{&pc}, &tail);
    const EarthAngle ea = earth_angle(tn);
    double wv[3], F[3];
    wind_eci_or_calm(r, ea, pp.shp, pp.chp, pp.inv_p, pp.wn, pp.we, wv);
    const double v[3] = {ve[0] * P.uv, ve[1] * P.uv, ve[2] * P.uv};
    aero_force(r, v, pp.rho, pp.inv_a, ea, wv, ph.area, tb, F);
    T = ph.thrust - ph.nozzle * pp.P;
    {
      const double Td[3] = {T * dir[0], T * dir[1], T * dir[2]};
      accel_parts(Td, F, inv_m, pp.g, inv_uv, tm, fc);
    }
    const double a[3] = {(v[0] + kOmega * r[1]) - wv[0], (v[1] - kOmega * r[0]) - wv[1], v[2] - wv[2]};
    const double s2 = a[0] * a[0] + a[1] * a[1] + a[2] * a[2];
    const double s = fsqrt(fmax(s2, 1.0e-200));
    const double mach = s * pp.inv_a;
    const double ca = interp_tab(mach, tb.ca, tb.cas, tb.Kc, 2, 1);
    const double cas = interp_tab_slope(mach, tb.ca, tb.cas, tb.Kc, 2);
    const double kk = (s2 > 0.0) ? 0.5 * pp.rho * ph.area * ca * s : 0.0;
    if (ph.air_fd) {
#pragma unroll
      for (int k = 0; k < 3; k++) {
        const double da[3] = {(k == 0) ? 1.0 : 0.0, (k == 1) ? 1.0 : 0.0, (k == 2) ? 1.0 : 0.0};
        double dF[3];
        aero_force_tangent(a, s2, s, pp.rho, pp.inv_a, ph.area, ca, cas, kk, da, 0.0, 0.0, dF);
#pragma unroll
        for (int c = 0; c < 3; c++) XPUT(ph.s_vv + 3 * k + c, ((c == k) ? djj : 0.0) - S * ((dF[c] * P.uv) * inv_m * inv_uv));
      }
    }
    double dsl[3], dcl[3], dalt[3], dh[3];
    geodetic_tangent(r, pp.inv_p, pc, dsl, dcl, dalt);
#pragma unroll
    for (int k = 0; k < 3; k++) dh[k] = (pc.G * pc.G) * dalt[k];
    const double Tk = pp.P / (pp.rho * tb.atm[33 + tail.k]);
    const AirTangent at = atmosphere_tangent(tail.h, Tk, pp.P, pp.rho, pp.inv_a, tb.atm);
    const bool in = tail.piece >= 0;
    const double s0 = in ? tb.winds[2 * tail.piece] : 0.0, s1 = in ? tb.winds[2 * tail.piece + 1] : 0.0;
    const double clon = (pp.inv_p > 0.0) ? r[0] * pp.inv_p : ea.c, slon = (pp.inv_p > 0.0) ? r[1] * pp.inv_p : ea.s;
    double dw[3][3];
    wind_eci_tangent(r, pp.inv_p, clon, slon, pc.sl, pc.cl, pp.wn, pp.we, s0, s1, dh, dsl, dcl, dw);
    double dg[3][3];
    gravity_tangent(r, P.barC20, dg);
#pragma unroll
    for (int k = 0; k < 3; k++) {
      const double da[3] = {((k == 1) ? kOmega : 0.0) - dw[k][0], ((k == 0) ? -kOmega : 0.0) - dw[k][1], -dw[k][2]};
      double dF[3];
      aero_force_tangent(a, s2, s, pp.rho, pp.inv_a, ph.area, ca, cas, kk, da, at.drho * dh[k], at.dinv_a * dh[k], dF);
      const double dT = -ph.nozzle * (at.dP * dh[k]);
#pragma unroll
      for (int c = 0; c < 3; c++) dfr[k][c] = ((dT * dir[c] + dF[c]) * inv_m + dg[k][c]) * inv_uv;
    }
  } else {
    T = ph.thrust;
    double gc[3];
    gravity_eci(r, P.barC20, gc);
#pragma unroll
    for (int c = 0; c < 3; c++) { tm[c] = (T * dir[c]) * inv_m; fc[c] = (tm[c] + gc[c]) * inv_uv; }
    double dg[3][3];
    gravity_tangent(r, P.barC20, dg);
#pragma unroll
    for (int k = 0; k < 3; k++)
#pragma unroll
      for (int c = 0; c < 3; c++) dfr[k][c] = dg[k][c] * inv_uv;
  }
#pragma unroll
  for (int k = 0; k < 3; k++)
#pragma unroll
    for (int c = 0; c < 3; c++) XPUT(kSlotVP + 3 * k + c, -S * (P.up * dfr[k][c]));
  {
    const double km = (P.um * inv_m) * (inv_uv * S);
#pragma unroll
    for (int c = 0; c < 3; c++) XPUT(kSlotVM + c, tm[c] * km);
  }
  {
    const double kqe = (T * inv_m) * (inv_uv * S);
#pragma unroll
    for (int k = 0; k < 4; k++) {
      const double a_ = (k < 2) ? -kqe : kqe;
      const double b_ = -2.0 * kqe;
      XPUT(ph.s_vq + 3 * k + 0, (2.0 * q[k]) * a_);
      XPUT(ph.s_vq + 3 * k + 1, q[3 - k] * b_);
      XPUT(ph.s_vq + 3 * k + 2, ((k & 1) ? q[k ^ 2] : -q[k ^ 2]) * b_);
    }
  }
#pragma unroll
  for (int c = 0; c < 3; c++) XPUT(ph.s_vt + c, fc[c] * hT);
#undef XPUT
  if (bad) *(volatile int32_t*)P.flag = 1;
}

hipError_t launch_eval_exact(const ProblemDev& P, int B, const double* d_x, double* d_jvar, hipStream_t s) {
  if (B <= 0) return hipSuccess;
  if (P.fd_recompute || !d_jvar) return hipErrorInvalidValue;
  const long long threads = (long long)B * P.N;
  const unsigned grid = (unsigned)((threads + kExactBlock - 1) / kExactBlock);
  const size_t lds = sizeof(double) * staged_table_doubles(P.Kw, P.Kc);
  hipLaunchKernelGGL(exact_jac_kernel, dim3(grid), dim3(kExactBlock), lds, s, P, B, d_x, d_jvar);
  return hipGetLastError();
}

}
```

gelato_amd/csrc/gel_kernels_exact_aero.hip:

```cpp
#include <hip/hip_runtime.h>

#include "gel_tables.h"
#include "gel_launch.h"
#include "gel_exact.h"

namespace gel {

constexpr int kExactAeroBlock = 256;

__global__ __launch_bounds__(kExactAeroBlock) void exact_aero_kernel(ProblemDev P, int nnodes, const AeroNodeDev* __restrict__ nodes,
                                                                      int B, const double* __restrict__ x, AeroLaunchOut O,
                                                                      long long ld, int sm) {
  extern __shared__ double lds[];
  const Tables tb = stage_tables(P, lds, true);
  const long long t = (long long)blockIdx.x * blockDim.x + threadIdx.x;
  if (t >= (long long)B * nnodes) return;
  const int b = (int)(t / nnodes), ni = (int)(t - (long long)b * nnodes);
  const AeroNodeDev Nd = nodes[ni];
  const PhaseDev ph = P.phases[Nd.phase];
  const int M = P.M, N = P.N, xi = ph.xa + Nd.k;
  const double* xb = x + (size_t)b * P.nvars;
  const double r[3] = {xb[M + 3 * xi] * P.up, xb[M + 3 * xi + 1] * P.up, xb[M + 3 * xi + 2] * P.up};
  const double v[3] = {xb[4 * M + 3 * xi] * P.uv, xb[4 * M + 3 * xi + 1] * P.uv, xb[4 * M + 3 * xi + 2] * P.uv};
  const double q[4] = {xb[7 * M + 4 * xi], xb[7 * M + 4 * xi + 1], xb[7 * M + 4 * xi + 2], xb[7 * M + 4 * xi + 3]};

  PosCentre pc;
  PosCentreTail tail;
  PosPart pp = pos_part<true, PosCentreSink, false>(r, tb, 0.0, nullptr, PosCentreSink{&pc}, &tail);
  pos_centre_tail(tail, pp.rho, pp.P, tb, pc, pp.wn, pp.we);
  const double to = xb[11 * M + 2 * N + Nd.phase], tf = xb[11 * M + 2 * N + Nd.phase + 1];
  const double tau = (Nd.k == 0) ? 0.0 : P.tau[ph.toff + Nd.k - 1];
  const EarthAngle ea = earth_angle(((Nd.k == 0) ? to : (tau * (tf - to) / 2 + (tf + to) / 2)) * P.ut);
  double w[3], a[3], dir[3];
  wind_eci_or_calm(r, ea, pp.shp, pp.chp, pp.inv_p, pp.wn, pp.we, w);
  const double nv2 = aero_vair2(r, v, w, a);
  thrust_dir(q, dir);
  const double ind = frsqrt(fmax(dir[0] * dir[0] + dir[1] * dir[1] + dir[2] * dir[2], 1.0e-300));
  const double cc = aero_cos(a, nv2, dir, ind);
  const double alpha = aero_acos(cc, nv2);
  const double qdyn = 0.5 * pp.rho * nv2;

  double dsl[3], dcl[3], dalt[3], dh[3];
  geodetic_tangent(r, pp.inv_p, pc, dsl, dcl, dalt);
#pragma unroll
  for (int k = 0; k < 3; k++) dh[k] = (pc.G * pc.G) * dalt[k];
  const double Tk = pp.P / (pp.rho * tb.atm[33 + tail.k]);
  const AirTangent at = atmosphere_tangent(tail.h, Tk, pp.P, pp.rho, pp.inv_a, tb.atm);
  const bool in = tail.piece >= 0;
  const double s0 = in ? tb.winds[2 * tail.piece] : 0.0, s1 = in ? tb.winds[2 * tail.piece + 1] : 0.0;
  const double clon = (pp.inv_p > 0.0) ? r[0] * pp.inv_p : ea.c, slon = (pp.inv_p > 0.0) ? r[1] * pp.inv_p : ea.s;
  double dw[3][3];
  wind_eci_tangent(r, pp.inv_p, clon, slon, pc.sl, pc.cl, pp.wn, pp.we, s0, s1, dh, dsl, dcl, dw);
  const double is = frsqrt(fmax(nv2, 1.0e-300));
  const double u[3] = {a[0] * is, a[1] * is, a[2] * is}, e[3] = {dir[0] * ind, dir[1] * ind, dir[2] * ind};
  double ep[3], upp[3];
#pragma unroll
  for (int c = 0; c < 3; c++) { ep[c] = e[c] - cc * u[c]; upp[c] = u[c] - cc * e[c]; }
  const double ne2 = ep[0] * ep[0] + ep[1] * ep[1] + ep[2] * ep[2], nu2 = upp[0] * upp[0] + upp[1] * upp[1] + upp[2] * upp[2];
  const bool has_da = (cc <= 1.0) && (nv2 >= 1.0e-12) && ne2 > 0.0 && nu2 > 0.0;
  const double kep = has_da ? frsqrt(ne2) * is : 0.0;
  const double kup = has_da ? frsqrt(nu2) * ind : 0.0;
#pragma unroll
  for (int c = 0; c < 3; c++) { ep[c] *= kep; upp[c] *= kup; }

  double* base[3];
  int32_t rowst[3];
#pragma unroll
  for (int kind = 0; kind < 3; kind++) {
    const int nq = (kind == 1) ? 0 : 4;
    const bool has = O.jac[kind] && Nd.row[kind] >= 0;
    const long long vs = ld ? ld : (long long)O.nrows[kind] * (8 + nq);
    base[kind] = has ? O.jac[kind] + (size_t)b * vs + (sm ? (size_t)Nd.row0[kind] : 0) + Nd.ko : nullptr;
    rowst[kind] = Nd.nk[kind];
  }
  const double il[3] = {frcp(Nd.limit[0]), frcp(Nd.limit[1]), frcp(Nd.limit[2])};
  bool bad = false;
#define EXPUT(bo, wd, col, dal, dq_)                                                                                   \
  do {                                                                                                                 \
    const double da_ = (dal), dqv_ = (dq_);                                                                            \
    _Pragma("unroll") for (int kind = 0; kind < 3; kind++) {                                                           \
      if (!base[kind] || ((bo) == 6 && kind == 1) || (sm && (bo) < 0)) continue;                                      \
      const double df_ = (kind == 0) ? da_ : ((kind == 1) ? dqv_ : qdyn * da_ + alpha * dqv_);                        \
      const double gv_ = ((bo) < 0) ? 0.0 : -(df_ * il[kind]);                                                       \
      const int nq_ = (kind == 1) ? 0 : 4, b_ = ((bo) < 0) ? 6 + nq_ : (bo);                                           \
      const size_t o_ = sm ? (size_t)(((bo) == 0 ? 1 : ((bo) == 3 ? 4 : 7)) + (col)) * rowst[kind]                     \
                           : (size_t)b_ * O.nrows[kind] + (size_t)(wd) * Nd.row0[kind] + (size_t)(col) * rowst[kind];  \
      base[kind][o_] = gv_;                                                                                            \
      bad = bad || !(fabs(gv_) <= 1.79769313486231570815e308);                                                         \
    }                                                                                                                  \
  } while (0)

#pragma unroll
  for (int k = 0; k < 3; k++) {
    const double da[3] = {((k == 1) ? kOmega : 0.0) - dw[k][0], ((k == 0) ? -kOmega : 0.0) - dw[k][1], -dw[k][2]};
    const double ada = a[0] * da[0] + a[1] * da[1] + a[2] * da[2];
    const double dq = pp.rho * ada + 0.5 * (at.drho * dh[k]) * nv2;
    const double dal = -(da[0] * ep[0] + da[1] * ep[1] + da[2] * ep[2]);
    EXPUT(0, 3, k, P.up * dal, P.up * dq);
  }
#pragma unroll
  for (int k = 0; k < 3; k++) EXPUT(3, 3, k, P.uv * -ep[k], P.uv * (pp.rho * a[k]));
#pragma unroll
  for (int k = 0; k < 4; k++) {
    const double dd[3] = {(k < 2) ? 2.0 * q[k] : -2.0 * q[k], 2.0 * q[3 - k], 2.0 * ((k & 1) ? q[k ^ 2] : -q[k ^ 2])};
    EXPUT(6, 4, k, -(dd[0] * upp[0] + dd[1] * upp[1] + dd[2] * upp[2]), 0.0);
  }
  EXPUT(-1, 2, 0, 0.0, 0.0);
  EXPUT(-1, 2, 1, 0.0, 0.0);
#undef EXPUT
  if (bad) *(volatile int32_t*)P.flag = 1;
}

hipError_t launch_aero_exact(const ProblemDev& P, int nnodes, const AeroNodeDev* nodes, int B, const double* d_x,
                             const AeroLaunchOut& out, hipStream_t s, long long ld, bool spec_major) {
  if (B <= 0 || nnodes <= 0) return hipSuccess;
  if (P.fd_recompute) return hipErrorInvalidValue;
  const long long threads = (long long)B * nnodes;
  const unsigned grid = (unsigned)((threads + kExactAeroBlock - 1) / kExactAeroBlock);
  const size_t lds = sizeof(double) * staged_table_doubles(P.Kw, P.Kc);
  hipLaunchKernelGGL(exact_aero_kernel, dim3(grid), dim3(kExactAeroBlock), lds, s, P, nnodes, nodes, B, d_x, out, ld,
                     (ld > 0 && spec_major) ? 1 : 0);
  return hipGetLastError();
}

}
```

gelato_amd/csrc/gel_rhs_parts.h:

```cpp
#pragma once
#include "gel_physics.h"

#ifndef GEL_CALM_SHORTCUT
#define GEL_CALM_SHORTCUT 1
#endif

namespace gel {

struct PosPart {
  double rho, P, inv_a;
  double wn, we;
  double g[3];
  double shp, chp;
  double inv_p;
};

GEL_DEV void geodetic_sincos(double x, double y, double z, double& sl, double& cl, double& p) {
  p = sqrt(x * x + y * y);
  const double a = z * kRa, b = p * kRb;
  const double ih = 1.0 / sqrt(a * a + b * b);
  const double st = a * ih, ct = b * ih;
  const double zz = z + kEp2 * kRb * (st * st * st);
  const double pp = p - kE2 * kRa * (ct * ct * ct);
  const double ihy = 1.0 / sqrt(zz * zz + pp * pp);
  sl = zz * ihy;
  cl = pp * ihy;
}

struct PosCentre {
  double p, ih, ihy;
  double sl, cl, icl;
  double N;
  double G;
  double s0, s1;
  double margin;
  AirCentre air;
};
enum PosCentreSlot { PCS_P = 0, PCS_IH, PCS_IHY, PCS_SL, PCS_CL, PCS_ICL, PCS_N, PCS_G, PCS_COUNT };
struct PosCentreTail { double h; int k, piece; };
struct NoSink { GEL_DEV void put(int, double) const {} };
struct PosCentreSink {
  PosCentre* pc;
  GEL_DEV void put(int i, double v) const {
    if (i == PCS_P) pc->p = v; else if (i == PCS_IH) pc->ih = v; else if (i == PCS_IHY) pc->ihy = v; else if (i == PCS_SL) pc->sl = v;
    else if (i == PCS_CL) pc->cl = v; else if (i == PCS_ICL) pc->icl = v; else if (i == PCS_N) pc->N = v; else pc->G = v;
  }
};

template <bool CENTRE = false, class Sink = NoSink, bool GRAV = true>
GEL_DEV PosPart pos_part(const double r[3], const Tables& tb, double barC20, Bracket2* wbr = nullptr, Sink sink = Sink(),
                         PosCentreTail* tail = nullptr) {
  PosPart o;
  double p, sl, cl;
  if (CENTRE) {
    double ih, ihy;
    geodetic_sincos_p(r[0], r[1], r[2], sl, cl, p, o.inv_p, &ih, &ihy);
    sink.put(PCS_IH, ih); sink.put(PCS_IHY, ihy); sink.put(PCS_P, p);
  } else geodetic_sincos_p(r[0], r[1], r[2], sl, cl, p, o.inv_p);
  {
    double irt;
    fsqrt_rsqrt(0.5 * (1.0 + cl), o.chp, irt);
    o.shp = (0.5 * sl) * irt;
  }
  const double N = fdiv(kRa, fsqrt(1.0 - kE2 * sl * sl));
  const double q = fdiv(p, cl);
  const double alt = q - N;
  if (CENTRE) {
    sink.put(PCS_SL, sl); sink.put(PCS_CL, cl); sink.put(PCS_N, N);
    sink.put(PCS_ICL, q * o.inv_p);
    sink.put(PCS_G, (alt < 86000.0) ? fdiv(6356766.0, 6356766.0 + alt) : 1.0);
  }
  const double h = geopotential_altitude(alt);
  const Air air = atmosphere(h, tb.atm);
  o.rho = air.rho; o.P = air.P; o.inv_a = air.inv_a;
  if (CENTRE) {
    wind_ned2_centre(h, tb.wind, tb.winds, tb.Kw, o.wn, o.we, tail->piece);
    tail->h = h; tail->k = us76_layer(h);
  } else if (wbr) wind_ned2_cached(h, tb.wind, tb.winds, tb.Kw, o.wn, o.we, *wbr);
  else wind_ned2(h, tb.wind, tb.winds, tb.Kw, o.wn, o.we);
  if (GRAV) gravity_eci(r, barC20, o.g);
  else o.g[0] = o.g[1] = o.g[2] = 0.0;
  return o;
}

GEL_DEV void pos_centre_tail(const PosCentreTail& t, double rho, double P, const Tables& tb, PosCentre& pc, double& wn, double& we) {
  double wm;
  wind_piece(t.h, t.piece, tb.wind, tb.winds, tb.Kw, wn, we, pc.s0, pc.s1, wm);
  const double lo = (t.k == 0) ? -1.0e300 : tb.atm[66 + t.k];
  const double hi = (t.k == 6) ? kGeopot86 : ((t.k < 10) ? tb.atm[67 + min(t.k, 9)] : 1.0e300);
  pc.margin = fmin(wm, fmin(t.h - lo, hi - t.h));
  pc.air.iT = rho * tb.atm[33 + t.k] * frcp(P);
  pc.air.h = t.h; pc.air.k = t.k;
}

GEL_DEV bool pos_delta(const double r[3], int kk, double dlt, const PosPart& c, const PosCentre& pc, const Tables& tb, PosPart& o) {
  const bool along_z = kk == 2;
  const double a = r[2] * kRa, b = pc.p * kRb;
  double u = 0.0, dp = 0.0, dh2, dst, dct, dih, ih1;
  o.inv_p = c.inv_p;
  if (!along_z) {
    const double xs = (kk == 0) ? r[0] : r[1];
    const double dp2 = dlt * __builtin_fma(2.0, xs, dlt);
    u = dp2 * c.inv_p * c.inv_p;
    dp = (0.5 * dp2 * c.inv_p) * (1.0 + u * (-0.25 + 0.125 * u));
    o.inv_p = c.inv_p * (1.0 + u * (-0.5 + 0.375 * u));
    const double db = dp * kRb;
    dh2 = db * __builtin_fma(2.0, b, db);
    const double uh = dh2 * pc.ih * pc.ih;
    dih = pc.ih * (uh * (-0.5 + 0.375 * uh));
    ih1 = pc.ih + dih;
    dst = a * dih;
    dct = db * ih1 + b * dih;
  } else {
    const double da = dlt * kRa;
    dh2 = da * __builtin_fma(2.0, a, da);
    const double uh = dh2 * pc.ih * pc.ih;
    dih = pc.ih * (uh * (-0.5 + 0.375 * uh));
    ih1 = pc.ih + dih;
    dst = da * ih1 + a * dih;
    dct = b * dih;
  }
  const double st = a * pc.ih, ct = b * pc.ih;
  const double dst3 = dst * (3.0 * st * (st + dst) + dst * dst);
  const double dct3 = dct * (3.0 * ct * (ct + dct) + dct * dct);
  const double dzz = along_z ? dlt + (kEp2 * kRb) * dst3 : (kEp2 * kRb) * dst3;
  const double dpp = along_z ? -((kE2 * kRa) * dct3) : dp - (kE2 * kRa) * dct3;
  const double e = (pc.cl * dpp + pc.sl * dzz) * pc.ihy;
  const double dlat = ((dzz * pc.cl - dpp * pc.sl) * pc.ihy) * (1.0 + e * (e - 1.0));
  const double hl2 = 0.5 * dlat * dlat;
  const double dsl = pc.cl * dlat - pc.sl * hl2, dcl = -(pc.sl * dlat + pc.cl * hl2);
  const double hd = 0.5 * dlat, hd2 = 0.5 * hd * hd;
  o.shp = c.shp + (c.chp * hd - c.shp * hd2);
  o.chp = c.chp - (c.shp * hd + c.chp * hd2);
  const double v = dcl * pc.icl;
  const double dq = ((dp - (pc.p * pc.icl) * dcl) * pc.icl) * (1.0 + v * (v - 1.0));
  const double nr = pc.N * (1.0 / kRa);
  const double uw = (-kE2 * dsl * __builtin_fma(2.0, pc.sl, dsl)) * (nr * nr);
  const double dN = pc.N * (uw * (-0.5 + 0.375 * uw));
  const double dalt = dq - dN;
  const double g1 = (pc.air.k <= 6) ? pc.G * (1.0 / 6356766.0) : 0.0;
  const double dh = (pc.G * pc.G) * dalt * (1.0 - dalt * g1);
  Air ca_;
  ca_.P = c.P; ca_.rho = c.rho; ca_.inv_a = c.inv_a; ca_.T = 0.0; ca_.a = 0.0;
  atmosphere_delta(ca_, pc.air, dh, tb.atm, o.P, o.rho, o.inv_a);
  o.wn = __builtin_fma(pc.s0, dh, c.wn);
  o.we = __builtin_fma(pc.s1, dh, c.we);
  return (c.inv_p > 0.0) && (fabs(u) < 1.0e-4) && (fabs(v) < 1.0e-4) && (fmax(fabs(dalt), fabs(dh)) < pc.margin);
}

struct EarthAngle { double c, s, ch, sh; };

struct EarthHalf { double ch, sh; };
GEL_DEV EarthAngle full_angle(const EarthHalf& h) {
  EarthAngle e;
  e.ch = h.ch; e.sh = h.sh;
  e.s = fresh_mul(2.0 * h.sh, h.ch);
  e.c = fresh_mul(h.ch - h.sh, h.ch + h.sh);
  return e;
}
GEL_DEV EarthAngle earth_angle(double t) {
  EarthAngle e;
  fsincos(kOmega * t / 2.0, &e.sh, &e.ch);
  e.s = 2.0 * e.sh * e.ch;
  e.c = (e.ch - e.sh) * (e.ch + e.sh);
  return e;
}

GEL_DEV void wind_eci(const double r[3], const EarthAngle& e, double s_hp, double c_hp, double inv_p, double wn,
                      double we, double w[3]) {
  const double px = r[0] * e.c + r[1] * e.s;
  const double py = -r[0] * e.s + r[1] * e.c;
  const double clon = (inv_p > 0.0) ? px * inv_p : 1.0, slon = py * inv_p;
  double th, ith;
  fsqrt_rsqrt(0.5 * (1.0 + fabs(clon)), th, ith);
  const double uh = (0.5 * slon) * ith;
  const double c_hl = (clon >= 0.0) ? th : fabs(uh);
  const double s_hl = (clon >= 0.0) ? uh : copysign(th, slon);
  const double irt2 = 0.70710678118654752440;
  const double b0 = c_hl * (c_hp - s_hp) * irt2, b1 = s_hl * (c_hp + s_hp) * irt2;
  const double b2 = -c_hl * (c_hp + s_hp) * irt2, b3 = s_hl * (c_hp - s_hp) * irt2;
  const double q0 = e.ch * b0 - e.sh * b3;
  const double q1 = -(e.ch * b1 - e.sh * b2);
  const double q2 = -(e.ch * b2 + e.sh * b1);
  const double q3 = -(e.ch * b3 + e.sh * b0);
  const double t0 = -wn * q1 - we * q2;
  const double t1 = wn * q0 + we * q3;
  const double t2 = -wn * q3 + we * q0;
  const double t3 = wn * q2 - we * q1;
  w[0] = q0 * t1 - q1 * t0 - q2 * t3 + q3 * t2;
  w[1] = q0 * t2 + q1 * t3 - q2 * t0 - q3 * t1;
  w[2] = q0 * t3 - q1 * t2 + q2 * t1 - q3 * t0;
}

GEL_DEV void wind_eci_or_calm(const double r[3], const EarthAngle& e, double s_hp, double c_hp, double inv_p, double wn,
                              double we, double w[3]) {
#if GEL_CALM_SHORTCUT
  if (__builtin_amdgcn_ballot_w64(!(wn == 0.0 && we == 0.0)) == 0) {
    w[0] = 0.0; w[1] = 0.0; w[2] = 0.0;
    return;
  }
#endif
  wind_eci(r, e, s_hp, c_hp, inv_p, wn, we, w);
}

#ifndef GEL_AERO_ROTATE
#define GEL_AERO_ROTATE 0
#endif
GEL_DEV void aero_force(const double r[3], const double v[3], double rho, double inv_a_sound, const EarthAngle& e,
                        const double w[3], double area, const Tables& tb, double F[3], Bracket* br = nullptr) {
  const double d0 = v[0] + kOmega * r[1];
  const double d1 = v[1] - kOmega * r[0];
#if GEL_AERO_ROTATE
  const double e0 = d0 * e.c + d1 * e.s;
  const double e1 = -d0 * e.s + d1 * e.c;
  const double a0 = (e0 * e.c - e1 * e.s) - w[0];
  const double a1 = (e0 * e.s + e1 * e.c) - w[1];
#else
  const double a0 = d0 - w[0];
  const double a1 = d1 - w[1];
#endif
  const double a2 = v[2] - w[2];
  const double vn = fsqrt(fmax(a0 * a0 + a1 * a1 + a2 * a2, 1.0e-200));
  const double mach = vn * inv_a_sound;
  const double ca = br ? interp_tab_cached(mach, tb.ca, tb.cas, tb.Kc, 2, 1, *br) : interp_tab(mach, tb.ca, tb.cas, tb.Kc, 2, 1);
  const double k = 0.5 * rho * area * ca * vn;
  F[0] = k * -a0; F[1] = k * -a1; F[2] = k * -a2;
}

GEL_DEV void accel(const double Td[3], const double F[3], double inv_m, const double g[3], double inv_uv,
                   double out[3]) {
#pragma unroll
  for (int c = 0; c < 3; c++) out[c] = ((Td[c] + F[c]) * inv_m + g[c]) * inv_uv;
}
GEL_DEV void accel_parts(const double Td[3], const double F[3], double inv_m, const double g[3], double inv_uv, double tm[3],
                         double out[3]) {
#pragma unroll
  for (int c = 0; c < 3; c++) { tm[c] = (Td[c] + F[c]) * inv_m; out[c] = (tm[c] + g[c]) * inv_uv; }
}
GEL_DEV void accel_noair(const double Td[3], double inv_m, const double g[3], double inv_uv, double out[3]) {
#pragma unroll
  for (int c = 0; c < 3; c++) out[c] = (Td[c] * inv_m + g[c]) * inv_uv;
}

GEL_DEV void thrust_dir(const double q[4], double dir[3]) {
  dir[0] = q[0] * q[0] + q[1] * q[1] - q[2] * q[2] - q[3] * q[3];
  dir[1] = q[0] * q[3] + q[1] * q[2] + q[2] * q[1] + q[3] * q[0];
  dir[2] = -q[0] * q[2] + q[1] * q[3] - q[2] * q[0] + q[3] * q[1];
}

GEL_DEV void quat_rate(const double q[4], double u0, double u1, double unit_u, double dq[4]) {
  const double d2r = 0.017453292519943295769;
  const double oy = (u0 * unit_u) * d2r, oz = (u1 * unit_u) * d2r;
  dq[0] = 0.5 * (-q[2] * oy - q[3] * oz);
  dq[1] = 0.5 * (q[2] * oz - q[3] * oy);
  dq[2] = 0.5 * (q[0] * oy - q[1] * oz);
  dq[3] = 0.5 * (q[0] * oz + q[1] * oy);
}

GEL_DEV double aero_vair2(const double r[3], const double v[3], const double w[3], double a[3]) {
  a[0] = (v[0] + kOmega * r[1]) - w[0]; a[1] = (v[1] - kOmega * r[0]) - w[1]; a[2] = v[2] - w[2];
  return a[0] * a[0] + a[1] * a[1] + a[2] * a[2];
}
GEL_DEV double aero_cos(const double a[3], double nv2, const double d[3], double ind) {
  return ((a[0] * d[0] + a[1] * d[1] + a[2] * d[2]) * frsqrt(fmax(nv2, 1.0e-300))) * ind;
}
GEL_DEV double aero_acos(double c, double nv2) { return (c > 1.0) ? 0.0 : ((nv2 < 1.0e-12) ? 0.0 : acos(c)); }
GEL_DEV bool aero_dalpha(double c_p, double nv2_p, double c_c, double inv_s, bool centre_ok, double& t) {
  const double t0 = (c_c - c_p) * inv_s, k = (0.5 * c_c) * inv_s;
  const double t1 = t0 - (k * t0) * t0;
  t = (t0 - (k * t1) * t1) + (t1 * t1) * (t1 * (1.0 / 6.0));
  return centre_ok && (c_p <= 1.0) && (nv2_p >= 1.0e-12) && (fabs(k * t0) < 1.0e-4);
}


}
```

gelato_amd/csrc/gel_section_rhs.h:

```cpp
#pragma once
#include "gel_tables.h"

namespace gel {

GEL_DEV void section_rhs(const ProblemDev& P, const PhaseDev& ph, const Tables& tb, double vp, double sig, double to, double tf,
                         const double xt[11], double u0, double u1, double F[11]) {
  F[0] = ph.engine_on ? ph.mf_um : 0.0;
#pragma unroll
  for (int c = 0; c < 3; c++) F[1 + c] = xt[4 + c] * vp;
  const double m = xt[0] * P.um;
  const double r[3] = {xt[1] * P.up, xt[2] * P.up, xt[3] * P.up};
  const double q[4] = {xt[7], xt[8], xt[9], xt[10]};
  double dir[3], f[3];
  thrust_dir(q, dir);
  if (ph.air) {
    const double v3[3] = {xt[4] * P.uv, xt[5] * P.uv, xt[6] * P.uv};
    const PosPart pp = pos_part(r, tb, P.barC20);
    const EarthAngle ea = earth_angle(sig * (tf - to) / 2 + (tf + to) / 2);
    double w[3], Fa[3];
    wind_eci_or_calm(r, ea, pp.shp, pp.chp, pp.inv_p, pp.wn, pp.we, w);
    aero_force(r, v3, pp.rho, pp.inv_a, ea, w, ph.area, tb, Fa);
    const double T = ph.thrust - ph.nozzle * pp.P;
    const double Td[3] = {T * dir[0], T * dir[1], T * dir[2]};
    accel(Td, Fa, 1.0 / m, pp.g, P.inv_uv, f);
  } else {
    double g[3];
    gravity_eci(r, P.barC20, g);
    const double Td[3] = {ph.thrust * dir[0], ph.thrust * dir[1], ph.thrust * dir[2]};
    accel_noair(Td, 1.0 / m, g, P.inv_uv, f);
  }
#pragma unroll
  for (int c = 0; c < 3; c++) F[4 + c] = f[c];
  double dq[4] = {0.0, 0.0, 0.0, 0.0};
  if (!ph.hold) quat_rate(q, u0, u1, P.uu, dq);
#pragma unroll
  for (int c = 0; c < 4; c++) F[7 + c] = dq[c];
}

}
```

Before: 21.71 million.

## Compute wind directly in inertial frame from latitude, skipping Earth-angle quaternion

Adds a GEL_WIND_LOCAL path, enabled by default, that computes the wind vector directly from geodetic sin/cos latitude and the position's longitude direction. This avoids computing the Earth rotation angle and half-angle quaternion chain on every residual and Jacobian wind evaluation. The full ECI quaternion form is kept only as a lane-masked fallback for polar points where inv_p is not positive. The change threads sl/cl through PosPart, the park slots and the finite-difference sweeps. It drops the half-latitude sqrt and the earth_angle trig in the common case, at the cost of extra ballot branches and different rounding.

```diff
diff --git a/gelato_amd/csrc/gel_eval_kernel.h b/gelato_amd/csrc/gel_eval_kernel.h
--- a/gelato_amd/csrc/gel_eval_kernel.h
+++ b/gelato_amd/csrc/gel_eval_kernel.h
@@ -886,6 +886,22 @@
     EMIT_GROUP(3, kSlotVM, vm_, CG_VM, 0, false, true);                                                                \
   } while (0)
     if (ph.air) {
+#if GEL_WIND_LOCAL
+      const EarthAngle no_ea{1.0, 0.0, 1.0, 0.0};
+      const auto defect_ea = [&]() {
+        int jl_ = jc;
+        if (AERO) asm volatile("" : "+v"(jl_));
+        const double tau_ = P.tau[ph.toff + jl_];
+        return earth_angle(tau_ * (tf - to) / 2 + (tf + to) / 2);
+      };
+      const auto aero_ea = [&]() {
+        int jl_ = jc;
+        asm volatile("" : "+v"(jl_));
+        const double tau_ = P.tau[ph.toff + jl_];
+        return earth_angle((tau_ * (tf - to) / 2 + (tf + to) / 2) * P.ut);
+      };
+      (void)tn;
+#else
       EarthHalf eh{1.0, 0.0};
       bool have_eh = false;
 #define GEL_NEED_EARTH_ANGLE(wn_, we_)                                                                                 \
@@ -898,14 +914,17 @@
       eh.ch = e_.ch; eh.sh = e_.sh; have_eh = true;                                                                    \
     }                                                                                                                  \
   } while (0)
+#endif
       PosCentreTail pt;
       double cen_rho = 0.0, cen_P = 0.0, cen_inv_a = 0.0;
       double dir2 = 0.0;
+#if !GEL_WIND_LOCAL
       EarthHalf aeh{1.0, 0.0};
       bool have_aeh = false;
 #ifndef GEL_AEH
 #define GEL_AEH aeh
 #endif
+#endif
 #ifndef GEL_X_NOPOS
 #define GEL_X_NOPOS 0
 #endif
@@ -917,6 +936,7 @@
 #endif
       const bool aero_on = AERO && akinds != 0;
       const bool a_need_alpha = AERO && (akinds & 5) != 0;
+#if !GEL_WIND_LOCAL
 #define GEL_AERO_NEED_EA(wn_, we_)                                                                                     \
   do {                                                                                                                 \
     if (!have_aeh && __builtin_amdgcn_ballot_w64(!((wn_) == 0.0 && (we_) == 0.0)) != 0) {                               \
@@ -927,6 +947,7 @@
       aeh.ch = e_.ch; aeh.sh = e_.sh; have_aeh = true;                                                                 \
     }                                                                                                                  \
   } while (0)
+#endif
 #define GEL_AERO_FETCH()                                                                                               \
   const int ab_[3] = {load_const(&aph->base[0]), load_const(&aph->base[1]), load_const(&aph->base[2])};                \
   const double ax_[3] = {load_const(&aph->ilx[0]), load_const(&aph->ilx[1]), load_const(&aph->ilx[2])};                \
@@ -970,6 +991,11 @@
         const double r[3] = {fresh_product(re[0], P.up), fresh_product(re[1], P.up), fresh_product(re[2], P.up)};
         if (JAC) pp = pos_part<true, ParkSink>(r, tb, P.barC20, nullptr, ParkSink{park}, &pt);
         else pp = pos_part(r, tb, P.barC20);
+#if GEL_WIND_LOCAL
+        const EarthAngle ea = no_ea;
+        const bool cen_polar = __builtin_amdgcn_ballot_w64(!(pp.inv_p > 0.0)) != 0;
+        wind_local_or_calm(r, pp.sl, pp.cl, pp.inv_p, pp.wn, pp.we, defect_ea, w);
+#else
         if (__builtin_amdgcn_ballot_w64(!(pp.wn == 0.0 && pp.we == 0.0)) != 0) {
           const EarthAngle e0 = earth_angle(tn);
           eh.ch = e0.ch; eh.sh = e0.sh; have_eh = true;
@@ -977,6 +1003,7 @@
         }
         const EarthAngle ea = full_angle(eh);
         wind_eci_or_calm(r, ea, pp.shp, pp.chp, pp.inv_p, pp.wn, pp.we, w);
+#endif
 #pragma unroll
         for (int c = 0; c < 3; c++) v[c] = PARK_GET(PK_V0 + c) * P.uv;
         aero_force(r, v, pp.rho, pp.inv_a, ea, w, ph.area, tb, F, GEL_CA_BRACKET);
@@ -1011,7 +1038,9 @@
         }
         if (JAC) {
           asm volatile("" ::: "memory");
+#if !GEL_WIND_LOCAL
           PARK_SET(PK_LV0, pp.shp); PARK_SET(PK_LV1, pp.chp);
+#endif
           if (!AERO) PARK_SET(PK_LV2, pp.inv_p);
         }
         if (JAC && lead && !P.fd_recompute) GEL_MASS_CLOSED(tm);
@@ -1068,6 +1097,17 @@
           double va[3], wa[3], a0[3];
 #pragma unroll
           for (int c = 0; c < 3; c++) va[c] = PARK_GET(PK_V0 + c) * P.uv;
+#if GEL_WIND_LOCAL
+#pragma unroll
+          for (int c = 0; c < 3; c++) wa[c] = w[c];
+          if (cen_polar) {
+            PosCentre pcx;
+            double wn_, we_, p_, ip_, ih_;
+            pos_centre_tail(pt, pp.rho, pp.P, tb, pcx, wn_, we_);
+            geodetic_p_ih(ra[0], ra[1], ra[2], p_, ip_, ih_);
+            wind_polar_lanes(ra, PARK_GET(PK_FP0 + PCS_SL), PARK_GET(PK_FP0 + PCS_CL), ip_, wn_, we_, aero_ea, wa);
+          }
+#else
           if (have_eh) {
             const EarthAngle e1 = earth_angle(PARK_GET(PK_ACC) * P.ut);
             aeh.ch = e1.ch; aeh.sh = e1.sh; have_aeh = true;
@@ -1081,6 +1121,7 @@
           } else {
             wa[0] = 0.0; wa[1] = 0.0; wa[2] = 0.0;
           }
+#endif
           const double nv2 = aero_vair2(ra, va, wa, a0);
           const double ind = frsqrt(fmax(dir[0] * dir[0] + dir[1] * dir[1] + dir[2] * dir[2], 1.0e-300));
           const double cc = a_need_alpha ? aero_cos(a0, nv2, dir, ind) : 0.0;
@@ -1133,12 +1174,20 @@
       }
       if (JAC && (!SPLIT || part)) {
         const int k0 = SPLIT ? part - 1 : 0, k1 = SPLIT ? part : 3;
-#define GEL_POS_SWEEP_F(rp, pq, f_)                                                                           \
-  do {                                                                                                        \
-    double wq_[3], Fp_[3];                                                                                    \
+#if GEL_WIND_LOCAL
+#define GEL_POS_SWEEP_WIND(rp, pq, wq_)                                                                       \
+    const EarthAngle ea = no_ea;                                                                              \
+    wind_local_or_calm(rp, (pq).sl, (pq).cl, (pq).inv_p, (pq).wn, (pq).we, defect_ea, wq_)
+#else
+#define GEL_POS_SWEEP_WIND(rp, pq, wq_)                                                                       \
     GEL_NEED_EARTH_ANGLE((pq).wn, (pq).we);                                                                   \
     const EarthAngle ea = full_angle(eh);                                                                     \
-    wind_eci_or_calm(rp, ea, (pq).shp, (pq).chp, (pq).inv_p, (pq).wn, (pq).we, wq_);                          \
+    wind_eci_or_calm(rp, ea, (pq).shp, (pq).chp, (pq).inv_p, (pq).wn, (pq).we, wq_)
+#endif
+#define GEL_POS_SWEEP_F(rp, pq, f_, wq_)                                                                      \
+  do {                                                                                                        \
+    double Fp_[3];                                                                                            \
+    GEL_POS_SWEEP_WIND(rp, pq, wq_);                                                                          \
     const double vq_[3] = {PARK_GET(PK_V0) * P.uv, PARK_GET(PK_V1) * P.uv, PARK_GET(PK_V2) * P.uv};           \
     aero_force(rp, vq_, (pq).rho, (pq).inv_a, ea, wq_, ph.area, tb, Fp_, GEL_CA_BRACKET);                     \
     const double Tp_ = ph.thrust - ph.nozzle * (pq).P;                                                        \
@@ -1150,11 +1199,19 @@
     const double vp_[3] = {FDQ((f_)[0], PARK_GET(PK_Q0)), FDQ((f_)[1], PARK_GET(PK_Q1)), FDQ((f_)[2], PARK_GET(PK_Q2))}; \
     EMIT_GROUP(3, kSlotVP + 3 * (kk), vp_, CG_VP, kk, false, okl_);                                           \
   } while (0)
-#define GEL_AERO_POS(kk, rp, pq, okl_)                                                                        \
+#if GEL_WIND_LOCAL
+#define GEL_AERO_POS_WIND(rp, pq, wd_, wq_)    \
+    _Pragma("unroll") for (int c_ = 0; c_ < 3; c_++) wq_[c_] = (wd_)[c_];                                     \
+    wind_polar_lanes(rp, (pq).sl, (pq).cl, (pq).inv_p, (pq).wn, (pq).we, aero_ea, wq_)
+#else
+#define GEL_AERO_POS_WIND(rp, pq, wd_, wq_)                                                                   \
+    GEL_AERO_NEED_EA((pq).wn, (pq).we);                                                                       \
+    wind_eci_or_calm(rp, full_angle(GEL_AEH), (pq).shp, (pq).chp, (pq).inv_p, (pq).wn, (pq).we, wq_)
+#endif
+#define GEL_AERO_POS(kk, rp, pq, okl_, wd_)                                                                   \
   do {                                                                                                        \
     double wq_[3], a_[3];                                                                                     \
-    GEL_AERO_NEED_EA((pq).wn, (pq).we);                                                                       \
-    wind_eci_or_calm(rp, full_angle(GEL_AEH), (pq).shp, (pq).chp, (pq).inv_p, (pq).wn, (pq).we, wq_);             \
+    GEL_AERO_POS_WIND(rp, pq, wd_, wq_);                                                                      \
     const double vq_[3] = {PARK_GET(PK_V0) * P.uv, PARK_GET(PK_V1) * P.uv, PARK_GET(PK_V2) * P.uv};           \
     const double nv2_ = aero_vair2(rp, vq_, wq_, a_);                                                         \
     const double dd_[3] = {PARK_GET(PK_Q3), PARK_GET(PK_DJJ), dir2};                                          \
@@ -1166,6 +1223,11 @@
     GEL_AERO_FETCH();                                                                                         \
     GEL_AERO_ENTRY(0, kk, a_, nv2_, dd_, ind_, (pq).rho, okl_, cc_, fabs(acs_), PARK_GET(PK_AQC), isc_, !__builtin_signbit(acs_)); \
   } while (0)
+#if GEL_WIND_LOCAL
+#define GEL_LOAD_HALF_LAT(pc, pcv) pcv.sl = pc.sl; pcv.cl = pc.cl
+#else
+#define GEL_LOAD_HALF_LAT(pc, pcv) pcv.shp = PARK_GET(PK_LV0); pcv.chp = PARK_GET(PK_LV1)
+#endif
 #define GEL_LOAD_POS_CENTRE(pc, pcv)                                                                                   \
   PosCentre pc;                                                                                                        \
   pc.ihy = PARK_GET(PK_FP0 + PCS_IHY);                                                                                 \
@@ -1173,7 +1235,7 @@
   pc.N = PARK_GET(PK_FP0 + PCS_N); pc.G = PARK_GET(PK_FP0 + PCS_G);                                                    \
   PosPart pcv;                                                                                                         \
   pcv.rho = cen_rho; pcv.P = cen_P; pcv.inv_a = cen_inv_a;                                                             \
-  pcv.shp = PARK_GET(PK_LV0); pcv.chp = PARK_GET(PK_LV1);                                                              \
+  GEL_LOAD_HALF_LAT(pc, pcv);                                                                                          \
   if (AERO) {                                                                                                          \
     geodetic_p_ih(fresh_product(re[0], P.up), fresh_product(re[1], P.up), fresh_product(re[2], P.up), pc.p, pcv.inv_p, pc.ih); \
   } else {                                                                                                             \
@@ -1202,10 +1264,10 @@
               if (__builtin_amdgcn_ballot_w64(ok) == 0) continue;
             }
             gravity_eci(rp, P.barC20, pq.g);
-            double f[3];
-            GEL_POS_SWEEP_F(rp, pq, f);
+            double f[3], wq[3];
+            GEL_POS_SWEEP_F(rp, pq, f, wq);
             GEL_POS_SWEEP_EMIT(k, f, ok);
-            if (aero_on && !GEL_X_NOPOS) GEL_AERO_POS(k, rp, pq, ok);
+            if (aero_on && !GEL_X_NOPOS) GEL_AERO_POS(k, rp, pq, ok, wq);
           }
         }
         if (todo) {
@@ -1228,13 +1290,16 @@
             }
             asm volatile("" ::: "memory");
             PosPart pq = pos_part(rp, tb, P.barC20);
-            double f[3];
-            GEL_POS_SWEEP_F(rp, pq, f);
+            double f[3], wq[3];
+            GEL_POS_SWEEP_F(rp, pq, f, wq);
             GEL_POS_SWEEP_EMIT(k, f, !ok);
-            if (aero_on && !GEL_X_NOPOS) GEL_AERO_POS(k, rp, pq, !ok);
+            if (aero_on && !GEL_X_NOPOS) GEL_AERO_POS(k, rp, pq, !ok, wq);
           }
         }
 #undef GEL_AERO_POS
+#undef GEL_AERO_POS_WIND
+#undef GEL_POS_SWEEP_WIND
+#undef GEL_LOAD_HALF_LAT
 #undef GEL_LOAD_POS_CENTRE
 #undef GEL_NEED_EARTH_ANGLE
 #undef GEL_AERO_NEED_EA
@@ -1253,7 +1318,12 @@
           const double r[3] = {fresh_product(re[0], P.up), fresh_product(re[1], P.up), fresh_product(re[2], P.up)};
           const PosPart p2 = pos_part(r, tb, P.barC20);
           const double T2 = ph.thrust - ph.nozzle * p2.P;
-          PARK_SET(PK_FP0, p2.shp); PARK_SET(PK_FP1, p2.chp); PARK_SET(PK_FP2, p2.inv_p); PARK_SET(PK_FP3, p2.wn); PARK_SET(PK_FP4, p2.we);
+#if GEL_WIND_LOCAL
+          PARK_SET(PK_FP0, p2.sl); PARK_SET(PK_FP1, p2.cl); PARK_SET(PK_FP2, p2.inv_p);
+#else
+          PARK_SET(PK_FP0, p2.shp); PARK_SET(PK_FP1, p2.chp); PARK_SET(PK_FP2, p2.inv_p);
+#endif
+          PARK_SET(PK_FP3, p2.wn); PARK_SET(PK_FP4, p2.we);
           PARK_SET(PK_FP5, p2.rho); PARK_SET(PK_FP6, p2.inv_a);
           PARK_SET(PK_LV0, p2.g[0]); PARK_SET(PK_LV1, p2.g[1]); PARK_SET(PK_LV2, p2.g[2]);
           PARK_SET(PK_Q0, T2 * PARK_GET(PK_Q3)); PARK_SET(PK_Q1, T2 * PARK_GET(PK_DJJ)); PARK_SET(PK_Q2, T2 * dir2);
@@ -1264,10 +1334,16 @@
           const double to_p = (k == 0) ? to + dx : to;
           const double tf_p = (k == 1) ? tf + dx : tf;
           const double tnp = tau2 * (tf_p - to_p) / 2 + (tf_p + to_p) / 2;
-          const EarthAngle eq = earth_angle(tnp);
           double wq[3], Fp[3], f[3];
           const double rq[3] = {re[0] * P.up, re[1] * P.up, re[2] * P.up};
+#if GEL_WIND_LOCAL
+          const EarthAngle eq = no_ea;
+          wind_local_or_calm(rq, PARK_GET(PK_FP0), PARK_GET(PK_FP1), PARK_GET(PK_FP2), PARK_GET(PK_FP3), PARK_GET(PK_FP4),
+                             [&]() { return earth_angle(tnp); }, wq);
+#else
+          const EarthAngle eq = earth_angle(tnp);
           wind_eci_or_calm(rq, eq, PARK_GET(PK_FP0), PARK_GET(PK_FP1), PARK_GET(PK_FP2), PARK_GET(PK_FP3), PARK_GET(PK_FP4), wq);
+#endif
           const double vq[3] = {PARK_GET(PK_V0) * P.uv, PARK_GET(PK_V1) * P.uv, PARK_GET(PK_V2) * P.uv};
           aero_force(rq, vq, PARK_GET(PK_FP5), PARK_GET(PK_FP6), eq, wq, ph.area, tb, Fp, GEL_CA_BRACKET);
           const double Tq[3] = {PARK_GET(PK_Q0), PARK_GET(PK_Q1), PARK_GET(PK_Q2)};
diff --git a/gelato_amd/csrc/gel_kernels.hip b/gelato_amd/csrc/gel_kernels.hip
--- a/gelato_amd/csrc/gel_kernels.hip
+++ b/gelato_amd/csrc/gel_kernels.hip
@@ -113,7 +113,7 @@
   const PosPart pp = pos_part(r, tb, A.barC20);
   const EarthAngle ea = earth_angle(A.t[i]);
   double w[3], F[3], dir[3], f[3];
-  wind_eci(r, ea, pp.shp, pp.chp, pp.inv_p, pp.wn, pp.we, w);
+  wind_eci(r, ea, pp, w);
   aero_force(r, v, pp.rho, pp.inv_a, ea, w, A.area, tb, F);
   thrust_dir(q, dir);
   const double T = A.thrust - A.nozzle * pp.P;
@@ -345,6 +345,15 @@
 #define AP_SET(i, v) (park[(i) * 64] = (v))
   PosCentre pc;
   PosPart pp;
+#if GEL_WIND_LOCAL
+  const auto aero_ea = [&]() {
+    const int kn_ = nodes[ni].k, phn_ = nodes[ni].phase;
+    const double to_ = xb[11 * M + 2 * N + phn_], tf_ = xb[11 * M + 2 * N + phn_ + 1];
+    const double tau_ = (kn_ == 0) ? 0.0 : P.tau[P.phases[phn_].toff + kn_ - 1];
+    return earth_angle(((kn_ == 0) ? to_ : (tau_ * (tf_ - to_) / 2 + (tf_ + to_) / 2)) * P.ut);
+  };
+#define GEL_AERO_WIND(rp_, pq_, w_) wind_local_or_calm(rp_, (pq_).sl, (pq_).cl, (pq_).inv_p, (pq_).wn, (pq_).we, aero_ea, w_)
+#else
   EarthAngle ea{1.0, 0.0, 1.0, 0.0};
   bool have_ea = false;
 #define GEL_AERO_NEED_EA(wn_, we_)                                                                                     \
@@ -358,6 +367,12 @@
       have_ea = true;                                                                                                  \
     }                                                                                                                  \
   } while (0)
+#define GEL_AERO_WIND(rp_, pq_, w_)                                                                                    \
+  do {                                                                                                                 \
+    GEL_AERO_NEED_EA((pq_).wn, (pq_).we);                                                                              \
+    wind_eci_or_calm(rp_, ea, (pq_).shp, (pq_).chp, (pq_).inv_p, (pq_).wn, (pq_).we, w_);                              \
+  } while (0)
+#endif
   double chk = 0.0;
   {
     double r[3], v[3], q[4], w[3], a0[3], dir[3];
@@ -368,8 +383,7 @@
     PosCentreTail pt;
     pp = pos_part<true, PosCentreSink, false>(r, tb, 0.0, nullptr, PosCentreSink{&pc}, &pt);
     pos_centre_tail(pt, pp.rho, pp.P, tb, pc, pp.wn, pp.we);
-    GEL_AERO_NEED_EA(pp.wn, pp.we);
-    wind_eci_or_calm(r, ea, pp.shp, pp.chp, pp.inv_p, pp.wn, pp.we, w);
+    GEL_AERO_WIND(r, pp, w);
     const double nv2 = aero_vair2(r, v, w, a0);
     thrust_dir(q, dir);
     const double ind = frsqrt(fmax(dir[0] * dir[0] + dir[1] * dir[1] + dir[2] * dir[2], 1.0e-300));
@@ -454,11 +468,11 @@
         const double tau2 = (kn == 0) ? 0.0 : P.tau[P.phases[phn].toff + kn - 1];
         const double to_p = (c == 0) ? to2 + dx : to2, tf_p = (c == 1) ? tf2 + dx : tf2;
         const double tp = ((kn == 0) ? to_p : (tau2 * (tf_p - to_p) / 2 + (tf_p + to_p) / 2)) * P.ut;
-        const EarthAngle eq = earth_angle(tp);
         const double r[3] = {fresh_product(re[0], P.up), fresh_product(re[1], P.up), fresh_product(re[2], P.up)};
         const double vq[3] = {xb[4 * M + 3 * xi] * P.uv, xb[4 * M + 3 * xi + 1] * P.uv, xb[4 * M + 3 * xi + 2] * P.uv};
         double wq[3], aq[3];
-        wind_eci(r, eq, pp.shp, pp.chp, pp.inv_p, pp.wn, pp.we, wq);
+        const EarthAngle eq = earth_angle(tp);
+        wind_eci(r, eq, pp, wq);
         const double nvq = aero_vair2(r, vq, wq, aq);
         const double dq[3] = {AP_GET(AP_DIR), AP_GET(AP_DIR + 1), AP_GET(AP_DIR + 2)};
         GEL_AERO_EMIT(-1, 2, c, aq, nvq, dq, AP_GET(AP_IND), pp.rho, false, false, false);
@@ -470,8 +484,7 @@
 #define GEL_AERO_POS_TAIL(c, rp, pq, skip_)                                                          \
   do {                                                                                               \
     double wq_[3], a_[3];                                                                            \
-    GEL_AERO_NEED_EA((pq).wn, (pq).we);                                                              \
-    wind_eci_or_calm(rp, ea, (pq).shp, (pq).chp, (pq).inv_p, (pq).wn, (pq).we, wq_);                 \
+    GEL_AERO_WIND(rp, pq, wq_);                                                                      \
     const double vq_[3] = {xb[4 * M + 3 * xi] * P.uv, xb[4 * M + 3 * xi + 1] * P.uv, xb[4 * M + 3 * xi + 2] * P.uv}; \
     const double nv2_ = aero_vair2(rp, vq_, wq_, a_);                                                \
     const double dd_[3] = {AP_GET(AP_DIR), AP_GET(AP_DIR + 1), AP_GET(AP_DIR + 2)};                  \
@@ -548,6 +561,7 @@
   }
 #undef GEL_AERO_EMIT
 #undef GEL_AERO_NEED_EA
+#undef GEL_AERO_WIND
 #undef AP_AIDX
 #undef AP_GET
 #undef AP_SET
diff --git a/gelato_amd/csrc/gel_kernels_exact.hip b/gelato_amd/csrc/gel_kernels_exact.hip
--- a/gelato_amd/csrc/gel_kernels_exact.hip
+++ b/gelato_amd/csrc/gel_kernels_exact.hip
@@ -80,7 +80,7 @@
     const PosPart pp = pos_part<true, PosCentreSink>(r, tb, P.barC20, nullptr, PosCentreSink{&pc}, &tail);
     const EarthAngle ea = earth_angle(tn);
     double wv[3], F[3];
-    wind_eci_or_calm(r, ea, pp.shp, pp.chp, pp.inv_p, pp.wn, pp.we, wv);
+    wind_eci_or_calm(r, ea, pp, wv);
     const double v[3] = {ve[0] * P.uv, ve[1] * P.uv, ve[2] * P.uv};
     aero_force(r, v, pp.rho, pp.inv_a, ea, wv, ph.area, tb, F);
     T = ph.thrust - ph.nozzle * pp.P;
diff --git a/gelato_amd/csrc/gel_kernels_exact_aero.hip b/gelato_amd/csrc/gel_kernels_exact_aero.hip
--- a/gelato_amd/csrc/gel_kernels_exact_aero.hip
+++ b/gelato_amd/csrc/gel_kernels_exact_aero.hip
@@ -32,7 +32,7 @@
   const double tau = (Nd.k == 0) ? 0.0 : P.tau[ph.toff + Nd.k - 1];
   const EarthAngle ea = earth_angle(((Nd.k == 0) ? to : (tau * (tf - to) / 2 + (tf + to) / 2)) * P.ut);
   double w[3], a[3], dir[3];
-  wind_eci_or_calm(r, ea, pp.shp, pp.chp, pp.inv_p, pp.wn, pp.we, w);
+  wind_eci_or_calm(r, ea, pp, w);
   const double nv2 = aero_vair2(r, v, w, a);
   thrust_dir(q, dir);
   const double ind = frsqrt(fmax(dir[0] * dir[0] + dir[1] * dir[1] + dir[2] * dir[2], 1.0e-300));
diff --git a/gelato_amd/csrc/gel_rhs_parts.h b/gelato_amd/csrc/gel_rhs_parts.h
--- a/gelato_amd/csrc/gel_rhs_parts.h
+++ b/gelato_amd/csrc/gel_rhs_parts.h
@@ -1,8 +1,12 @@
 #pragma once
 #include "gel_physics.h"
+#include "gel_wind.h"
 
 #ifndef GEL_CALM_SHORTCUT
 #define GEL_CALM_SHORTCUT 1
+#endif
+#ifndef GEL_AERO_ROTATE
+#define GEL_AERO_ROTATE 0
 #endif
 
 namespace gel {
@@ -11,7 +15,11 @@
   double rho, P, inv_a;
   double wn, we;
   double g[3];
+#if GEL_WIND_LOCAL
+  double sl, cl;
+#else
   double shp, chp;
+#endif
   double inv_p;
 };
 
@@ -57,11 +65,11 @@
     geodetic_sincos_p(r[0], r[1], r[2], sl, cl, p, o.inv_p, &ih, &ihy);
     sink.put(PCS_IH, ih); sink.put(PCS_IHY, ihy); sink.put(PCS_P, p);
   } else geodetic_sincos_p(r[0], r[1], r[2], sl, cl, p, o.inv_p);
-  {
-    double irt;
-    fsqrt_rsqrt(0.5 * (1.0 + cl), o.chp, irt);
-    o.shp = (0.5 * sl) * irt;
-  }
+#if GEL_WIND_LOCAL
+  o.sl = sl; o.cl = cl;
+#else
+  half_lat_pair(sl, cl, o.shp, o.chp);
+#endif
   const double N = fdiv(kRa, fsqrt(1.0 - kE2 * sl * sl));
   const double q = fdiv(p, cl);
   const double alt = q - N;
@@ -129,9 +137,13 @@
   const double dlat = ((dzz * pc.cl - dpp * pc.sl) * pc.ihy) * (1.0 + e * (e - 1.0));
   const double hl2 = 0.5 * dlat * dlat;
   const double dsl = pc.cl * dlat - pc.sl * hl2, dcl = -(pc.sl * dlat + pc.cl * hl2);
+#if GEL_WIND_LOCAL
+  o.sl = pc.sl + dsl; o.cl = pc.cl + dcl;
+#else
   const double hd = 0.5 * dlat, hd2 = 0.5 * hd * hd;
   o.shp = c.shp + (c.chp * hd - c.shp * hd2);
   o.chp = c.chp - (c.shp * hd + c.chp * hd2);
+#endif
   const double v = dcl * pc.icl;
   const double dq = ((dp - (pc.p * pc.icl) * dcl) * pc.icl) * (1.0 + v * (v - 1.0));
   const double nr = pc.N * (1.0 / kRa);
@@ -148,7 +160,6 @@
   return (c.inv_p > 0.0) && (fabs(u) < 1.0e-4) && (fabs(v) < 1.0e-4) && (fmax(fabs(dalt), fabs(dh)) < pc.margin);
 }
 
-struct EarthAngle { double c, s, ch, sh; };
 
 struct EarthHalf { double ch, sh; };
 GEL_DEV EarthAngle full_angle(const EarthHalf& h) {
@@ -166,32 +177,6 @@
   return e;
 }
 
-GEL_DEV void wind_eci(const double r[3], const EarthAngle& e, double s_hp, double c_hp, double inv_p, double wn,
-                      double we, double w[3]) {
-  const double px = r[0] * e.c + r[1] * e.s;
-  const double py = -r[0] * e.s + r[1] * e.c;
-  const double clon = (inv_p > 0.0) ? px * inv_p : 1.0, slon = py * inv_p;
-  double th, ith;
-  fsqrt_rsqrt(0.5 * (1.0 + fabs(clon)), th, ith);
-  const double uh = (0.5 * slon) * ith;
-  const double c_hl = (clon >= 0.0) ? th : fabs(uh);
-  const double s_hl = (clon >= 0.0) ? uh : copysign(th, slon);
-  const double irt2 = 0.70710678118654752440;
-  const double b0 = c_hl * (c_hp - s_hp) * irt2, b1 = s_hl * (c_hp + s_hp) * irt2;
-  const double b2 = -c_hl * (c_hp + s_hp) * irt2, b3 = s_hl * (c_hp - s_hp) * irt2;
-  const double q0 = e.ch * b0 - e.sh * b3;
-  const double q1 = -(e.ch * b1 - e.sh * b2);
-  const double q2 = -(e.ch * b2 + e.sh * b1);
-  const double q3 = -(e.ch * b3 + e.sh * b0);
-  const double t0 = -wn * q1 - we * q2;
-  const double t1 = wn * q0 + we * q3;
-  const double t2 = -wn * q3 + we * q0;
-  const double t3 = wn * q2 - we * q1;
-  w[0] = q0 * t1 - q1 * t0 - q2 * t3 + q3 * t2;
-  w[1] = q0 * t2 + q1 * t3 - q2 * t0 - q3 * t1;
-  w[2] = q0 * t3 - q1 * t2 + q2 * t1 - q3 * t0;
-}
-
 GEL_DEV void wind_eci_or_calm(const double r[3], const EarthAngle& e, double s_hp, double c_hp, double inv_p, double wn,
                               double we, double w[3]) {
 #if GEL_CALM_SHORTCUT
@@ -202,10 +187,61 @@
 #endif
   wind_eci(r, e, s_hp, c_hp, inv_p, wn, we, w);
 }
-
-#ifndef GEL_AERO_ROTATE
-#define GEL_AERO_ROTATE 0
-#endif
+GEL_DEV void pos_half_lat(const PosPart& o, double& shp, double& chp) {
+#if GEL_WIND_LOCAL
+  half_lat_pair(o.sl, o.cl, shp, chp);
+#else
+  shp = o.shp; chp = o.chp;
+#endif
+}
+GEL_DEV void wind_eci_or_calm(const double r[3], const EarthAngle& e, const PosPart& o, double w[3]) {
+  double shp, chp;
+  pos_half_lat(o, shp, chp);
+  wind_eci_or_calm(r, e, shp, chp, o.inv_p, o.wn, o.we, w);
+}
+GEL_DEV void wind_eci(const double r[3], const EarthAngle& e, const PosPart& o, double w[3]) {
+  double shp, chp;
+  pos_half_lat(o, shp, chp);
+  wind_eci(r, e, shp, chp, o.inv_p, o.wn, o.we, w);
+}
+
+template <class EA>
+GEL_DEV void wind_polar_lanes(const double r[3], double sl, double cl, double inv_p, double wn, double we, EA ea, double w[3]) {
+  if (__builtin_amdgcn_ballot_w64(!(inv_p > 0.0)) != 0) {
+#if GEL_CALM_SHORTCUT
+    if (__builtin_amdgcn_ballot_w64(!(wn == 0.0 && we == 0.0)) == 0) return;
+#endif
+    const EarthAngle e = ea();
+    double shp, chp, wq[3];
+    half_lat_pair(sl, cl, shp, chp);
+    wind_eci(r, e, shp, chp, inv_p, wn, we, wq);
+#pragma unroll
+    for (int c = 0; c < 3; c++) w[c] = (inv_p > 0.0) ? w[c] : wq[c];
+  }
+}
+template <class EA>
+GEL_DEV void wind_local_or_calm(const double r[3], double sl, double cl, double inv_p, double wn, double we, EA ea, double w[3]) {
+#if GEL_CALM_SHORTCUT
+  if (__builtin_amdgcn_ballot_w64(!(wn == 0.0 && we == 0.0)) == 0) {
+    w[0] = 0.0; w[1] = 0.0; w[2] = 0.0;
+    return;
+  }
+#endif
+  if (__builtin_amdgcn_ballot_w64(!(inv_p > 0.0)) != 0) {
+    double shp, chp, wq[3];
+    half_lat_pair(sl, cl, shp, chp);
+    wind_eci(r, ea(), shp, chp, inv_p, wn, we, wq);
+    wind_local(r, sl, cl, inv_p, wn, we, w);
+#pragma unroll
+    for (int c = 0; c < 3; c++) w[c] = (inv_p > 0.0) ? w[c] : wq[c];
+  } else {
+    wind_local(r, sl, cl, inv_p, wn, we, w);
+  }
+}
+#if GEL_WIND_LOCAL && GEL_AERO_ROTATE
+#error "GEL_WIND_LOCAL=1 forms no Earth angle off the polar axis: it needs GEL_AERO_ROTATE=0"
+#endif
+
 GEL_DEV void aero_force(const double r[3], const double v[3], double rho, double inv_a_sound, const EarthAngle& e,
                         const double w[3], double area, const Tables& tb, double F[3], Bracket* br = nullptr) {
   const double d0 = v[0] + kOmega * r[1];
diff --git a/gelato_amd/csrc/gel_section_rhs.h b/gelato_amd/csrc/gel_section_rhs.h
--- a/gelato_amd/csrc/gel_section_rhs.h
+++ b/gelato_amd/csrc/gel_section_rhs.h
@@ -18,7 +18,7 @@
     const PosPart pp = pos_part(r, tb, P.barC20);
     const EarthAngle ea = earth_angle(sig * (tf - to) / 2 + (tf + to) / 2);
     double w[3], Fa[3];
-    wind_eci_or_calm(r, ea, pp.shp, pp.chp, pp.inv_p, pp.wn, pp.we, w);
+    wind_eci_or_calm(r, ea, pp, w);
     aero_force(r, v3, pp.rho, pp.inv_a, ea, w, ph.area, tb, Fa);
     const double T = ph.thrust - ph.nozzle * pp.P;
     const double Td[3] = {T * dir[0], T * dir[1], T * dir[2]};
diff --git a/gelato_amd/csrc/gel_wind.h b/gelato_amd/csrc/gel_wind.h
--- /dev/null
+++ b/gelato_amd/csrc/gel_wind.h
@@ -0,0 +1,61 @@
+#pragma once
+
+#ifndef GEL_WIND_LOCAL
+#define GEL_WIND_LOCAL 1
+#endif
+
+namespace gel {
+
+struct EarthAngle { double c, s, ch, sh; };
+
+GEL_DEV void half_lat_pair(double sl, double cl, double& shp, double& chp) {
+  double irt;
+  fsqrt_rsqrt(0.5 * (1.0 + cl), chp, irt);
+  shp = (0.5 * sl) * irt;
+}
+
+GEL_DEV void wind_eci(const double r[3], const EarthAngle& e, double s_hp, double c_hp, double inv_p, double wn,
+                      double we, double w[3]) {
+  const double px = r[0] * e.c + r[1] * e.s;
+  const double py = -r[0] * e.s + r[1] * e.c;
+  const double clon = (inv_p > 0.0) ? px * inv_p : 1.0, slon = py * inv_p;
+  double th, ith;
+  fsqrt_rsqrt(0.5 * (1.0 + fabs(clon)), th, ith);
+  const double uh = (0.5 * slon) * ith;
+  const double c_hl = (clon >= 0.0) ? th : fabs(uh);
+  const double s_hl = (clon >= 0.0) ? uh : copysign(th, slon);
+  const double irt2 = 0.70710678118654752440;
+  const double b0 = c_hl * (c_hp - s_hp) * irt2, b1 = s_hl * (c_hp + s_hp) * irt2;
+  const double b2 = -c_hl * (c_hp + s_hp) * irt2, b3 = s_hl * (c_hp - s_hp) * irt2;
+  const double q0 = e.ch * b0 - e.sh * b3;
+  const double q1 = -(e.ch * b1 - e.sh * b2);
+  const double q2 = -(e.ch * b2 + e.sh * b1);
+  const double q3 = -(e.ch * b3 + e.sh * b0);
+  const double t0 = -wn * q1 - we * q2;
+  const double t1 = wn * q0 + we * q3;
+  const double t2 = -wn * q3 + we * q0;
+  const double t3 = wn * q2 - we * q1;
+  w[0] = q0 * t1 - q1 * t0 - q2 * t3 + q3 * t2;
+  w[1] = q0 * t2 + q1 * t3 - q2 * t0 - q3 * t1;
+  w[2] = q0 * t3 - q1 * t2 + q2 * t1 - q3 * t0;
+}
+
+GEL_DEV void wind_local(const double r[3], double sl, double cl, double inv_p, double wn, double we, double w[3]) {
+  const double cL = r[0] * inv_p, sL = r[1] * inv_p;
+  const double ns = wn * sl;
+  w[0] = -__builtin_fma(ns, cL, we * sL);
+  w[1] = __builtin_fma(we, cL, -(ns * sL));
+  w[2] = wn * cl;
+}
+
+GEL_DEV void wind_local_or_polar(const double r[3], const EarthAngle& e, double sl, double cl, double inv_p, double wn, double we,
+                                 double w[3]) {
+  wind_local(r, sl, cl, inv_p, wn, we, w);
+  if (!(inv_p > 0.0)) {
+    double shp, chp;
+    half_lat_pair(sl, cl, shp, chp);
+    wind_eci(r, e, shp, chp, inv_p, wn, we, w);
+  }
+}
+
+}
```

New measurement: 22.48 million, median of 6. +3.6%, better.
